# esteinig/sketchy

Measured on AMD Instinct MI355X. Metric: reads/sec streamed (s=10000,k=16,40k-genome ref), higher is better.
Workload: dtype u64

## Files before the change

include/sketchy_hip.h:

```cpp
#ifndef SKETCHY_HIP_H
#define SKETCHY_HIP_H

#include <stddef.h>
#include <stdint.h>

#ifdef __cplusplus
extern "C" {
#endif

#define SKX_OK 0
#define SKX_ERR_INVALID (-1)
#define SKX_ERR_NO_DEVICE (-2)
#define SKX_ERR_HIP (-3)
#define SKX_ERR_UNSORTED (-4)
#define SKX_ERR_CAPACITY (-5)
#define SKX_ERR_COMM (-6)
#define SKX_ERR_UNSUPPORTED (-7)

#define SKX_MAX_K 32u
#define SKX_MAX_TOP 64u
#define SKX_MAX_SPECIES 64u
#define SKX_MAX_FEATURES 64u
#define SKX_MAX_TABLE_SUM ((1ull << 54) - 1)

typedef struct skx_ref skx_ref;
typedef struct skx_stream skx_stream;
typedef struct skx_comm skx_comm;

const char *skx_last_error(void);
const char *skx_version(void);
int skx_device_count(void);
int skx_device_info(int device, char *name, size_t name_cap, int *compute_units, uint64_t *total_mem);
int skx_device_pci_bus_id(int device, char *bus_id, size_t cap);

#define SKX_COMM_TIMEOUT_EXIT 86
int skx_set_option(const char *name, uint64_t value);
int skx_get_option(const char *name, uint64_t *value);

int skx_ref_create(skx_ref **out, int device, uint32_t k, uint64_t seed, uint32_t s, uint32_t stride, uint32_t n_genomes,
                   const uint64_t *hashes, const uint32_t *col_len);
int skx_ref_create_multi(skx_ref **out, int device, uint32_t k, uint64_t seed, uint32_t s, uint32_t stride, uint32_t n_species,
                         const uint32_t *n_genomes, const uint64_t *const *hashes, const uint32_t *const *col_len);
int skx_ref_n_genomes(const skx_ref *ref, uint32_t *n_genomes);
int skx_ref_n_species(const skx_ref *ref, uint32_t *n_species);
int skx_ref_species_genomes(const skx_ref *ref, uint32_t species, uint32_t *n_genomes);
int skx_ref_sketch_size(const skx_ref *ref, uint32_t *s, uint32_t *stride);
int skx_ref_kmer_filter(const skx_ref *ref, uint64_t *n_keys, uint64_t *table_bytes);
int skx_ref_rare_index(const skx_ref *ref, uint64_t *n_keys, uint64_t *n_rare_keys, uint64_t *n_postings, uint64_t *bytes);
int skx_ref_patterns(const skx_ref *ref, uint64_t *n_long_lists, uint64_t *n_patterns, uint64_t *n_pattern_lists, uint64_t *bytes);
int skx_ref_static_dense(const skx_ref *ref, int *is_static, uint64_t *n_hashes);
int skx_ref_pass_bytes(const skx_ref *ref, uint64_t *bytes);
int skx_ref_set_genotypes(skx_ref *ref, uint32_t n_features, const uint32_t *codes);
int skx_ref_n_features(const skx_ref *ref, uint32_t *n_features);
void skx_ref_destroy(skx_ref *ref);

int skx_stream_create(skx_stream **out, const skx_ref *ref, uint32_t top_k, uint32_t max_batch_reads,
                      uint64_t max_batch_bases);
int skx_stream_push(skx_stream *st, const uint8_t *bases, const uint64_t *offsets, uint32_t n_reads,
                    uint32_t *topk_idx, uint64_t *topk_sum, uint32_t *per_read_shared, uint64_t *sketches,
                    uint32_t *sketch_len);
int skx_stream_push_device(skx_stream *st, const uint8_t *d_bases, const uint64_t *d_offsets, uint32_t n_reads,
                           uint64_t n_bases, uint32_t *d_topk_idx, uint64_t *d_topk_sum);
int skx_stream_enqueue_device(skx_stream *st, const uint8_t *d_bases, const uint64_t *d_offsets, uint32_t n_reads,
                              uint64_t n_bases, uint32_t *d_topk_idx, uint64_t *d_topk_sum);
int skx_stream_flush(skx_stream *st);
int skx_stream_set_packed_input(skx_stream *st, int on);
uint64_t skx_pack_bases(const uint8_t *ascii, uint64_t n, uint8_t *packed, uint64_t nibble_pos);
uint64_t skx_pack_line(const uint8_t *ascii, uint64_t n, uint8_t *packed, uint64_t nibble_pos, uint64_t *consumed);
int skx_stream_sync(skx_stream *st);
int skx_stream_submit(skx_stream *st, const uint8_t *bases, const uint64_t *offsets, uint32_t n_reads,
                      uint32_t *topk_idx, uint64_t *topk_sum, uint64_t *ticket);
int skx_stream_wait(skx_stream *st, uint64_t ticket);
int skx_stream_drain(skx_stream *st);
int skx_stream_bind_consensus(skx_stream *st, uint32_t *codes_out);
int skx_stream_bind_changes(skx_stream *st, uint32_t cap, uint32_t *n_events, uint32_t *ev_read, uint32_t *ev_idx, uint64_t *ev_sum,
                            uint32_t *ev_codes);
int skx_stream_table(skx_stream *st, uint64_t *cum);
int skx_stream_table_add(skx_stream *st, const uint64_t *add);
int skx_stream_reset(skx_stream *st);
int skx_stream_reads(const skx_stream *st, uint64_t *n_reads);
#define SKX_N_STATS 18
int skx_stream_stats(skx_stream *st, uint64_t *out, uint32_t n_out);
int skx_stream_rank(skx_stream *st, uint32_t top_k, uint32_t *idx, uint64_t *sum);
void skx_stream_destroy(skx_stream *st);

#define SKX_N_STAGES 5
int skx_stream_set_profiling(skx_stream *st, int enabled);
int skx_stream_profile(skx_stream *st, double *ms, uint64_t *launches);
int skx_stream_scan_alone(skx_stream *st, uint32_t reps, double *ms_avg);

int skx_sketch_reads(int device, uint32_t k, uint64_t seed, uint32_t s, const uint8_t *bases,
                     const uint64_t *offsets, uint32_t n_reads, uint64_t *sketches, uint32_t *sketch_len);
int skx_sketch_groups(int device, uint32_t k, uint64_t seed, uint32_t s, const uint8_t *bases, const uint64_t *offsets,
                      uint32_t n_records, const uint32_t *group_first, uint32_t n_groups,
                      uint64_t *sketches, uint32_t *sketch_len, uint64_t *valid_kmers);
int skx_sketch_groups_counts(int device, uint32_t k, uint64_t seed, uint32_t s, const uint8_t *bases, const uint64_t *offsets,
                             uint32_t n_records, const uint32_t *group_first, uint32_t n_groups, uint64_t *sketches,
                             uint32_t *sketch_len, uint64_t *valid_kmers, uint32_t *counts);
int skx_common_hashes(const skx_ref *ref, const uint64_t *query, const uint32_t *query_len, uint32_t n_query,
                      uint32_t q_stride, uint32_t *common);
int skx_rank_sketches(const skx_ref *ref, const uint64_t *query, const uint32_t *query_len, uint32_t n_query, uint32_t q_stride,
                      uint32_t top_k, uint32_t *top_idx, uint32_t *top_shared, uint32_t *common);
int skx_predict_groups(const skx_ref *ref, const uint8_t *bases, const uint64_t *offsets, uint32_t n_records,
                       const uint32_t *group_first, uint32_t n_groups, uint32_t top_k,
                       uint32_t *top_idx, uint32_t *top_shared, uint64_t *sketches, uint32_t *sketch_len, uint64_t *valid_kmers);
int skx_consensus_rows(const skx_ref *ref, const uint32_t *idx, uint64_t n_rows, uint32_t top_k, uint32_t *codes_out);

int skx_changes_rows(int device, const uint32_t *rows, uint64_t n_rows, uint32_t width, uint64_t cap, uint64_t *n_events,
                     uint64_t *ev_row);

#define SKX_COMM_ID_BYTES 128
int skx_comm_unique_id(uint8_t id[SKX_COMM_ID_BYTES]);
int skx_comm_create(skx_comm **out, int device, int rank, int n_ranks, const uint8_t id[SKX_COMM_ID_BYTES]);
int skx_comm_n_ranks(const skx_comm *comm, int *n_ranks);
int skx_stream_allreduce(skx_stream *st, skx_comm *comm);
void skx_comm_destroy(skx_comm *comm);

int skx_dev_malloc(int device, void **d_ptr, size_t bytes);
int skx_dev_free(int device, void *d_ptr);
int skx_dev_upload(int device, void *d_dst, const void *h_src, size_t bytes);
int skx_dev_download(int device, void *h_dst, const void *d_src, size_t bytes);
int skx_dev_synchronize(int device);
int skx_dev_mem_info(int device, uint64_t *free_bytes, uint64_t *total_bytes);
int skx_host_alloc(int device, void **h_ptr, size_t bytes);
int skx_host_free(int device, void *h_ptr);

#ifdef __cplusplus
}
#endif
#endif
```

sketchy_amd/_lib.py:

```python
import ctypes as C
import os

_HERE = os.path.dirname(os.path.abspath(__file__))
LIB_PATH = os.environ.get("SKX_LIB_PATH") or os.path.join(_HERE, "libsketchy_hip.so")

OK = 0
ERR_INVALID, ERR_NO_DEVICE, ERR_HIP, ERR_UNSORTED, ERR_CAPACITY, ERR_COMM, ERR_UNSUPPORTED = -1, -2, -3, -4, -5, -6, -7
N_STAGES = 5
STAGE_NAMES = ("sketch", "dictionary", "scan", "transpose", "rank")
COMM_ID_BYTES = 128
MAX_K = 32
MAX_TOP = 64
MAX_SPECIES = 64
MAX_FEATURES = 64
MAX_TABLE_SUM = (1 << 54) - 1

_vp, _u32, _u64, _i, _sz = C.c_void_p, C.c_uint32, C.c_uint64, C.c_int, C.c_size_t
_pp = C.POINTER(C.c_void_p)
SYMBOLS = [
    ("skx_last_error", C.c_char_p, []),
    ("skx_version", C.c_char_p, []),
    ("skx_device_count", _i, []),
    ("skx_device_info", _i, [_i, C.c_char_p, _sz, C.POINTER(_i), C.POINTER(_u64)]),
    ("skx_device_pci_bus_id", _i, [_i, C.c_char_p, _sz]),
    ("skx_set_option", _i, [C.c_char_p, _u64]),
    ("skx_get_option", _i, [C.c_char_p, C.POINTER(_u64)]),
    ("skx_ref_kmer_filter", _i, [_vp, C.POINTER(_u64), C.POINTER(_u64)]),
    ("skx_ref_rare_index", _i, [_vp, C.POINTER(_u64), C.POINTER(_u64), C.POINTER(_u64), C.POINTER(_u64)]),
    ("skx_ref_patterns", _i, [_vp, C.POINTER(_u64), C.POINTER(_u64), C.POINTER(_u64), C.POINTER(_u64)]),
    ("skx_ref_static_dense", _i, [_vp, C.POINTER(C.c_int), C.POINTER(_u64)]),
    ("skx_ref_create", _i, [_pp, _i, _u32, _u64, _u32, _u32, _u32, _vp, _vp]),
    ("skx_ref_create_multi", _i, [_pp, _i, _u32, _u64, _u32, _u32, _u32, _vp, _vp, _vp]),
    ("skx_ref_sketch_size", _i, [_vp, C.POINTER(_u32), C.POINTER(_u32)]),
    ("skx_ref_n_genomes", _i, [_vp, C.POINTER(_u32)]),
    ("skx_ref_n_species", _i, [_vp, C.POINTER(_u32)]),
    ("skx_ref_species_genomes", _i, [_vp, _u32, C.POINTER(_u32)]),
    ("skx_ref_pass_bytes", _i, [_vp, C.POINTER(_u64)]),
    ("skx_ref_set_genotypes", _i, [_vp, _u32, _vp]),
    ("skx_ref_n_features", _i, [_vp, C.POINTER(_u32)]),
    ("skx_ref_destroy", None, [_vp]),
    ("skx_stream_create", _i, [_pp, _vp, _u32, _u32, _u64]),
    ("skx_stream_push", _i, [_vp, _vp, _vp, _u32, _vp, _vp, _vp, _vp, _vp]),
    ("skx_stream_push_device", _i, [_vp, _vp, _vp, _u32, _u64, _vp, _vp]),
    ("skx_stream_enqueue_device", _i, [_vp, _vp, _vp, _u32, _u64, _vp, _vp]),
    ("skx_stream_flush", _i, [_vp]),
    ("skx_stream_set_packed_input", _i, [_vp, _i]),
    ("skx_pack_bases", _u64, [_vp, _u64, _vp, _u64]),
    ("skx_pack_line", _u64, [_vp, _u64, _vp, _u64, C.POINTER(_u64)]),
    ("skx_stream_sync", _i, [_vp]),
    ("skx_stream_submit", _i, [_vp, _vp, _vp, _u32, _vp, _vp, C.POINTER(_u64)]),
    ("skx_stream_wait", _i, [_vp, _u64]),
    ("skx_stream_drain", _i, [_vp]),
    ("skx_stream_bind_consensus", _i, [_vp, _vp]),
    ("skx_stream_bind_changes", _i, [_vp, _u32, _vp, _vp, _vp, _vp, _vp]),
    ("skx_stream_table", _i, [_vp, _vp]),
    ("skx_stream_table_add", _i, [_vp, _vp]),
    ("skx_stream_reset", _i, [_vp]),
    ("skx_stream_reads", _i, [_vp, C.POINTER(_u64)]),
    ("skx_stream_stats", _i, [_vp, C.POINTER(_u64), _u32]),
    ("skx_stream_rank", _i, [_vp, _u32, _vp, _vp]),
    ("skx_stream_destroy", None, [_vp]),
    ("skx_stream_set_profiling", _i, [_vp, _i]),
    ("skx_stream_profile", _i, [_vp, C.POINTER(C.c_double), C.POINTER(_u64)]),
    ("skx_stream_scan_alone", _i, [_vp, C.c_uint32, C.POINTER(C.c_double)]),
    ("skx_sketch_reads", _i, [_i, _u32, _u64, _u32, _vp, _vp, _u32, _vp, _vp]),
    ("skx_sketch_groups", _i, [_i, _u32, _u64, _u32, _vp, _vp, _u32, _vp, _u32, _vp, _vp, _vp]),
    ("skx_sketch_groups_counts", _i, [_i, _u32, _u64, _u32, _vp, _vp, _u32, _vp, _u32, _vp, _vp, _vp, _vp]),
    ("skx_common_hashes", _i, [_vp, _vp, _vp, _u32, _u32, _vp]),
    ("skx_rank_sketches", _i, [_vp, _vp, _vp, _u32, _u32, _u32, _vp, _vp, _vp]),
    ("skx_consensus_rows", _i, [_vp, _vp, _u64, _u32, _vp]),
    ("skx_changes_rows", _i, [_i, _vp, _u64, _u32, _u64, C.POINTER(_u64), _vp]),
    ("skx_predict_groups", _i, [_vp, _vp, _vp, _u32, _vp, _u32, _u32, _vp, _vp, _vp, _vp, _vp]),
    ("skx_comm_unique_id", _i, [_vp]),
    ("skx_comm_create", _i, [_pp, _i, _i, _i, _vp]),
    ("skx_comm_n_ranks", _i, [_vp, C.POINTER(_i)]),
    ("skx_stream_allreduce", _i, [_vp, _vp]),
    ("skx_comm_destroy", None, [_vp]),
    ("skx_dev_malloc", _i, [_i, _pp, _sz]),
    ("skx_dev_free", _i, [_i, _vp]),
    ("skx_dev_upload", _i, [_i, _vp, _vp, _sz]),
    ("skx_dev_download", _i, [_i, _vp, _vp, _sz]),
    ("skx_dev_synchronize", _i, [_i]),
# ... 34 lines not shown
```

sketchy_amd/api.py:

```python
import ctypes as C

import numpy as np

from . import _lib


def _p(a):
    return None if a is None else a.ctypes.data_as(C.c_void_p)


def pack_reads(bases, offsets, first_nibble=0):
    L = _lib.load()
    bases = np.ascontiguousarray(bases, np.uint8)
    offsets = np.ascontiguousarray(offsets, np.uint64)
    n = len(offsets) - 1
    packed = np.zeros((first_nibble + len(bases) + 1) // 2 + 1, np.uint8)
    out = np.zeros(n + 1, np.uint64)
    pos = int(first_nibble)
    out[0] = pos
    for r in range(n):
        a, b = int(offsets[r]), int(offsets[r + 1])
        if b > a:
            pos = int(L.skx_pack_bases(bases[a:b].ctypes.data_as(C.c_void_p), b - a, _p(packed), pos))
        out[r + 1] = pos
# ... 39 lines not shown
    for f in range(n_feat):
        col = [r[f] for r in rows]
        distinct = sorted(set(col), key=key)
        rank = {v: i for i, v in enumerate(distinct)}
        codes[:, f] = [rank[v] for v in col]
        values.append(distinct)
    return codes, values


class ReferenceSketch:

    def __init__(self, hashes, col_len=None, k=16, seed=0, device=0, s=None):
        L = _lib.load()
        many = isinstance(hashes, (list, tuple))
        mats = [np.ascontiguousarray(h, np.uint64) for h in (hashes if many else [hashes])]
        if any(m.ndim != 2 for m in mats) or len({m.shape[1] for m in mats}) != 1:
            raise ValueError("hashes must be [n_genomes, s] (one matrix per species, all with the same s)")
        lens = col_len if many else [col_len]
        lens = [None] * len(mats) if lens is None else list(lens)
        lens = [np.full(m.shape[0], m.shape[1], np.uint32) if c is None else np.ascontiguousarray(c, np.uint32)
                for m, c in zip(mats, lens)]
        self.species = [int(m.shape[0]) for m in mats]
        self.n_species = len(mats)
        self.n_genomes, self.stride = sum(self.species), int(mats[0].shape[1])
        self.s = self.stride if s is None else int(s)
        self.k, self.seed, self.device = int(k), int(seed), int(device)
        h = C.c_void_p()
        if self.n_species == 1:
            _lib.check(L.skx_ref_create(C.byref(h), device, self.k, self.seed, self.s, self.stride, self.n_genomes, _p(mats[0]), _p(lens[0])))
        else:
            ng = (C.c_uint32 * self.n_species)(*self.species)
            hp = (C.c_void_p * self.n_species)(*[m.ctypes.data for m in mats])
            cp = (C.c_void_p * self.n_species)(*[c.ctypes.data for c in lens])
            _lib.check(L.skx_ref_create_multi(C.byref(h), device, self.k, self.seed, self.s, self.stride, self.n_species, ng, hp, cp))
        self._h = h

    @property
    def kmer_filter(self):
        n, b = C.c_uint64(0), C.c_uint64(0)
        _lib.check(_lib.load().skx_ref_kmer_filter(self._h, C.byref(n), C.byref(b)))
        return n.value, b.value

    @property
    def rare_index(self):
        v = [C.c_uint64(0) for _ in range(4)]
        _lib.check(_lib.load().skx_ref_rare_index(self._h, *[C.byref(x) for x in v]))
        return dict(zip(("keys", "rare_keys", "postings", "bytes"), [x.value for x in v]))

    @property
    def patterns(self):
        v = [C.c_uint64(0) for _ in range(4)]
        _lib.check(_lib.load().skx_ref_patterns(self._h, *[C.byref(x) for x in v]))
        return dict(zip(("long_lists", "patterns", "pattern_lists", "bytes"), [x.value for x in v]))

    @property
    def static_dense(self):
        f, n = C.c_int(0), C.c_uint64(0)
        _lib.check(_lib.load().skx_ref_static_dense(self._h, C.byref(f), C.byref(n)))
        return bool(f.value), n.value

    @property
    def pass_bytes(self) -> int:
        b = C.c_uint64(0)
        _lib.check(_lib.load().skx_ref_pass_bytes(self._h, C.byref(b)))
        return b.value

    def common_hashes(self, query, query_len=None) -> np.ndarray:
        query = np.ascontiguousarray(query, np.uint64)
        nq, stride = query.shape
        query_len = np.full(nq, stride, np.uint32) if query_len is None else np.ascontiguousarray(query_len, np.uint32)
        out = np.zeros((nq, self.n_genomes), np.uint32)
        _lib.check(_lib.load().skx_common_hashes(self._h, _p(query), _p(query_len), nq, stride, _p(out)))
        return out

    def rank_sketches(self, query, query_len=None, top=1, want_common=False):
        query = np.ascontiguousarray(query, np.uint64)
        if query.ndim != 2:
            raise ValueError("query must be [n_query, stride]")
        nq, stride = query.shape
        query_len = np.full(nq, stride, np.uint32) if query_len is None else np.ascontiguousarray(query_len, np.uint32)
        if query_len.shape != (nq,):
            raise ValueError("query_len must hold one length per query row")
        top = int(top)
        idx = np.zeros((nq, self.n_species, max(top, 0)), np.uint32)
        shared = np.zeros_like(idx)
        common = np.zeros((nq, self.n_genomes), np.uint32) if want_common else None
        if stride == 0:
            if query_len.any():
                raise ValueError("query_len exceeds the stride of the query rows")
            query, stride = np.zeros((max(nq, 1), 1), np.uint64), 1
        _lib.check(_lib.load().skx_rank_sketches(self._h, _p(query), _p(query_len), nq, stride, top, _p(idx), _p(shared),
                                                 _p(common) if want_common else None))
        return (idx, shared, common) if want_common else (idx, shared)

    def predict_groups(self, bases, offsets, group_first, top=1, want_sketches=False, want_valid_kmers=False):
        bases = np.ascontiguousarray(bases, np.uint8)
        offsets = np.ascontiguousarray(offsets, np.uint64)
        group_first = np.ascontiguousarray(group_first, np.uint32)
        if offsets.ndim != 1 or len(offsets) < 1 or group_first.ndim != 1 or len(group_first) < 1:
            raise ValueError("offsets and group_first are 1-D with at least one entry")
        n, ng = len(offsets) - 1, len(group_first) - 1
        top = int(top)
        idx = np.zeros((ng, self.n_species, max(top, 0)), np.uint32)
        shared = np.zeros_like(idx)
        sk = np.zeros((ng, self.s), np.uint64) if want_sketches else None
        sl = np.zeros(ng, np.uint32) if want_sketches else None
# ... 112 lines not shown

    def flush(self):
        _lib.check(_lib.load().skx_stream_flush(self._h))

    def set_packed_input(self, on=True):
        _lib.check(_lib.load().skx_stream_set_packed_input(self._h, int(bool(on))))

    def sync(self):
        _lib.check(_lib.load().skx_stream_sync(self._h))

    def submit(self, h_bases, h_offsets, n_reads, h_topk_idx=None, h_topk_sum=None, consensus=None, changes=None) -> int:
        self._bind(consensus, changes)
        t = C.c_uint64(0)
        _lib.check(_lib.load().skx_stream_submit(self._h, h_bases, h_offsets, n_reads, h_topk_idx, h_topk_sum, C.byref(t)))
        return t.value

    def wait(self, ticket):
        _lib.check(_lib.load().skx_stream_wait(self._h, ticket))

    def drain(self):
        _lib.check(_lib.load().skx_stream_drain(self._h))

    def table(self) -> np.ndarray:
        cum = np.zeros(self.ref.n_genomes, np.uint64)
        _lib.check(_lib.load().skx_stream_table(self._h, _p(cum)))
        return cum

    def table_add(self, add):
        add = np.ascontiguousarray(add, np.uint64)
        assert len(add) == self.ref.n_genomes
        _lib.check(_lib.load().skx_stream_table_add(self._h, _p(add)))

    def reset(self):
        _lib.check(_lib.load().skx_stream_reset(self._h))

    @property
    def reads(self) -> int:
        n = C.c_uint64(0)
        _lib.check(_lib.load().skx_stream_reads(self._h, C.byref(n)))
        return n.value

    def rank(self, top=None):
        top = self.top if top is None else int(top)
        shape = (top,) if self.ref.n_species == 1 else (self.ref.n_species, top)
        idx, sm = np.zeros(shape, np.uint32), np.zeros(shape, np.uint64)
        _lib.check(_lib.load().skx_stream_rank(self._h, top, _p(idx), _p(sm)))
        return idx, sm

    def consensus(self, top=None) -> np.ndarray:
        idx, _ = self.rank(top)
        return self.ref.consensus_rows(idx)

    def stats(self):
        v = (C.c_uint64 * 18)()
        _lib.check(_lib.load().skx_stream_stats(self._h, v, 18))
        names = ("last_pairs", "last_passes", "dictionary_size", "reads_block_sketcher", "passes", "passes_lean_scan",
                 "pair_capacity", "live_rank_groups", "reads_split_over_waves", "read_segments", "row_pool_grown",
                 "passes_shared", "groups_unshared", "query_rows", "query_rows_grown", "dictionary_dense", "batches_compact", "batches_full")
        return dict(zip(names, [int(x) for x in v]))

    def set_profiling(self, on=True):
        _lib.check(_lib.load().skx_stream_set_profiling(self._h, int(on)))

    def profile(self):
        ms = (C.c_double * _lib.N_STAGES)()
        n = (C.c_uint64 * _lib.N_STAGES)()
        _lib.check(_lib.load().skx_stream_profile(self._h, ms, n))
        return {name: dict(ms=ms[i], launches=int(n[i])) for i, name in enumerate(_lib.STAGE_NAMES)}

    def scan_alone(self, reps=3) -> float:
        ms = C.c_double(0)
        _lib.check(_lib.load().skx_stream_scan_alone(self._h, int(reps), C.byref(ms)))
        return ms.value

    def allreduce(self, comm):
        _lib.check(_lib.load().skx_stream_allreduce(self._h, comm._h))

    def close(self):
        if getattr(self, "_h", None):
            _lib.load().skx_stream_destroy(self._h)
            self._h = None

    def __del__(self):
        try:
            self.close()
        except Exception:
            pass


class Comm:

    @staticmethod
    def unique_id() -> bytes:
        buf = (C.c_uint8 * _lib.COMM_ID_BYTES)()
        _lib.check(_lib.load().skx_comm_unique_id(buf))
        return bytes(buf)

    def __init__(self, device, rank, n_ranks, uid: bytes):
        buf = (C.c_uint8 * _lib.COMM_ID_BYTES).from_buffer_copy(uid)
        h = C.c_void_p()
        _lib.check(_lib.load().skx_comm_create(C.byref(h), device, rank, n_ranks, buf))
        self._h = h

    @property
    def n_ranks(self) -> int:
        n = C.c_int(0)
        _lib.check(_lib.load().skx_comm_n_ranks(self._h, C.byref(n)))
        return n.value

    def close(self):
        if getattr(self, "_h", None):
# ... 92 lines not shown
```

sketchy_amd/csrc/skx_capi.hip:

```cpp
#include <dlfcn.h>
#include <hip/hip_runtime.h>
#include <rccl/rccl.h>

#include <unistd.h>

#include <algorithm>
#include <atomic>
#include <chrono>
#include <cmath>
#include <condition_variable>
#include <cstdarg>
#include <cstdio>
#include <cstdlib>
#include <cstring>
#include <mutex>
#include <string>
#include <thread>
#include <unordered_map>
#include <vector>

#include "sketchy_hip.h"
#include "skx_common.hpp"
#include "skx_kernels.hpp"

// ... 184 lines not shown
        return SKX_OK;
    }
    return fail(SKX_ERR_INVALID, "unknown option '%s'", name);
}
SKX_API int skx_get_option(const char* name, uint64_t* value) {
    if (!name || !value) return fail(SKX_ERR_INVALID, "NULL argument");
    if (!strcmp(name, "kmer_prefilter")) { *value = g_kmer_prefilter; return SKX_OK; }
    if (!strcmp(name, "filter_bits_per_hash")) { *value = g_filter_bits_per_hash; return SKX_OK; }
    if (!strcmp(name, "stream_query_rows")) { *value = g_stream_query_rows; return SKX_OK; }
    if (!strcmp(name, "stream_coalesce")) { *value = g_stream_coalesce; return SKX_OK; }
    if (!strcmp(name, "comm_timeout_ms")) { *value = g_comm_timeout_ms; return SKX_OK; }
    if (!strcmp(name, "rank_lanes")) { *value = g_rank_lanes; return SKX_OK; }
    if (!strcmp(name, "rare_hash_genomes")) { *value = g_rare_hash_genomes; return SKX_OK; }
    if (!strcmp(name, "reuse_membership")) { *value = g_reuse_membership; return SKX_OK; }
    return fail(SKX_ERR_INVALID, "unknown option '%s'", name);
}

struct skx_ref {
    int device = 0;
    u32 k = 0, s = 0 , s_read = 0 ;
    u32 n_genomes = 0 , n_tiles = 0, n_pad = 0, rb = 0, n_bands = 0;
    u64 seed = 0;
    u32 n_species = 0;
    std::vector<u32> sp_n, sp_g0, sp_real0;
    u32 min_species = 0;
    u32 max_species = 0;
    u32 *d_sp_g0 = nullptr, *d_sp_n = nullptr, *d_grp_sp = nullptr;
    u32* d_real2pad = nullptr;
    u64* d_mat = nullptr;
    u64 *d_lo = nullptr, *d_hi = nullptr;
    u64 max_ref = 0;
    bool any = false;
    u32 n_exc = 0;
    u32* d_exc_g = nullptr;
    u64* d_exc_h = nullptr;
    u64* d_filt = nullptr;
    u32 filt_shift = 0;
    u64 filt_bits = 0, n_distinct = 0;
    u32* d_kf = nullptr;
    u32 kf_shift = 0, kf_keys = 0;
    u64* d_kt_key = nullptr;
    u32 *d_kt_cnt = nullptr, *d_kt_off = nullptr, *d_post = nullptr;
    u32 kt_mask = 0, rare_max = 0;
    u64 n_keys = 0, n_rare_keys = 0, n_postings = 0;
    u64* d_mlong = nullptr;
    u64* d_mlongT = nullptr;
    u32 *d_lid = nullptr, *d_lslot = nullptr;
    u64 n_long = 0;
    u32 n_lw = 0;
    u32 *d_prec = nullptr, *d_pat_rep = nullptr, *d_npat = nullptr;
    u64* d_pm = nullptr;
    u32 n_pat = 0;
    u64 n_pat_lists = 0;
    bool rare_direct = false;
    u64* d_qs = nullptr;
    u32* d_nsd = nullptr;
    u32* d_win_s = nullptr;
    u32 n_sd = 0;
    bool static_dense = false;
    u32* d_srow = nullptr;
    u32* d_seg = nullptr;
    u32* d_segw = nullptr;
    u32 sd_tail0 = 0;
    u64 n_forced_rare = 0;
    u32* d_codes = nullptr;
    u32 n_features = 0;
    skx::RareIndex rare_index() const {
        skx::RareIndex ri{d_kt_key, d_kt_off, d_kt_cnt, d_post, kt_mask, d_mlong, d_lid, d_lslot, n_pad / 64, d_mlongT, n_lw};
        ri.prec = d_prec; ri.pat_rep = d_pat_rep; ri.pm = d_pm; ri.d_npat = d_npat; ri.n_pat = n_pat;
        if (static_dense) { ri.qs = d_qs; ri.n_sd = n_sd; ri.srow = d_srow; ri.tail0 = sd_tail0; }
        return ri;
    }
    skx::KmerFilter kmer_filter() const { return skx::KmerFilter{d_kf, kf_shift}; }
    skx::Species species() const { return skx::Species{d_sp_g0, d_sp_n, d_grp_sp, n_species}; }
};

static void ref_free(skx_ref* r) {
    if (!r) return;
    (void)hipSetDevice(r->device);
    (void)hipFree(r->d_mat); (void)hipFree(r->d_lo); (void)hipFree(r->d_hi);
    (void)hipFree(r->d_exc_g); (void)hipFree(r->d_exc_h); (void)hipFree(r->d_filt); (void)hipFree(r->d_kf);
    (void)hipFree(r->d_sp_g0); (void)hipFree(r->d_sp_n); (void)hipFree(r->d_grp_sp); (void)hipFree(r->d_real2pad);
    (void)hipFree(r->d_kt_key); (void)hipFree(r->d_kt_cnt); (void)hipFree(r->d_kt_off); (void)hipFree(r->d_post);
    (void)hipFree(r->d_mlong); (void)hipFree(r->d_mlongT); (void)hipFree(r->d_lid); (void)hipFree(r->d_lslot);
    (void)hipFree(r->d_prec); (void)hipFree(r->d_pat_rep); (void)hipFree(r->d_npat); (void)hipFree(r->d_pm);
    (void)hipFree(r->d_qs); (void)hipFree(r->d_nsd); (void)hipFree(r->d_win_s);
    (void)hipFree(r->d_srow); (void)hipFree(r->d_seg); (void)hipFree(r->d_segw); (void)hipFree(r->d_codes);
    delete r;
}

static const u32 kGroupGenomes = skx::kRankWords * 64u;

static const u32 kPatMax = 16384;
static const u32 kPatGroupMin = 4;
static void build_patterns(skx_ref* r) {
    static const int pat_env = skx::knob("SKX_PATTERNS") ? atoi(skx::knob("SKX_PATTERNS")) : 1;
    if (!pat_env || !r->d_mlong || r->n_long < 64 || r->n_long >= 0x7FFFFFFFull) return;
    const u32 n_long = (u32)r->n_long, n_gw = r->n_pad / 64;
    u32 *d_sig = nullptr, *d_pat_of = nullptr, *d_done = nullptr;
    u64* d_content = nullptr;
    auto drop = [&]() {
        (void)hipFree(r->d_prec); (void)hipFree(r->d_pat_rep); (void)hipFree(r->d_npat); (void)hipFree(r->d_pm);
        r->d_prec = r->d_pat_rep = r->d_npat = nullptr; r->d_pm = nullptr; r->n_pat = 0; r->n_pat_lists = 0;
        (void)hipGetLastError();
    };
    bool ok = hipMalloc(&d_sig, (size_t)n_long * 4) == hipSuccess && hipMalloc(&d_content, (size_t)n_long * 8) == hipSuccess;
    try {
        std::vector<u32> sig(n_long), pat_of(n_long, 0xFFFFFFFFu), rep;
        std::vector<u64> content(n_long);
        if (ok) {
            skx::launch_list_sig(nullptr, r->d_lslot, n_long, r->d_kt_off, r->d_kt_cnt, r->d_post, d_sig, d_content);
            ok = hipGetLastError() == hipSuccess && hipMemcpy(sig.data(), d_sig, (size_t)n_long * 4, hipMemcpyDeviceToHost) == hipSuccess &&
                 hipMemcpy(content.data(), d_content, (size_t)n_long * 8, hipMemcpyDeviceToHost) == hipSuccess;
        }
        if (ok) {
            struct Exact { u32 count = 0, first = 0, sig = 0; };
            struct Group { u32 size = 0, best_count = 0, best_first = 0; };
            std::unordered_map<u64, Exact> exact;
            std::unordered_map<u32, Group> groups;
            exact.reserve(n_long);
            for (u32 i = 0; i < n_long; ++i) {
                Exact& e = exact[content[i] ^ ((u64)sig[i] * 0xD6E8FEB86659FD93ull)];
                if (!e.count) { e.first = i; e.sig = sig[i]; }
                e.count += 1;
                groups[sig[i]].size += 1;
            }
            for (const auto& kv : exact) {
                const Exact& e = kv.second;
                Group& g = groups[e.sig];
                if (e.count > g.best_count || (e.count == g.best_count && e.first < g.best_first)) { g.best_count = e.count; g.best_first = e.first; }
            }
            std::vector<std::pair<u32, u32>> order;
            for (const auto& kv : groups) if (kv.second.size >= kPatGroupMin) order.push_back({kv.second.size, kv.first});
            std::sort(order.begin(), order.end(), [](const std::pair<u32, u32>& a, const std::pair<u32, u32>& b) { return a.first != b.first ? a.first > b.first : a.second < b.second; });
            if (order.size() > kPatMax) order.resize(kPatMax);
            std::unordered_map<u32, u32> pat_of_sig;
            for (const auto& o : order) { pat_of_sig[o.second] = (u32)rep.size(); rep.push_back(groups[o.second].best_first); }
            for (u32 i = 0; i < n_long; ++i) { const auto it = pat_of_sig.find(sig[i]); if (it != pat_of_sig.end()) pat_of[i] = it->second; }
            ok = !rep.empty();
        }
        const u32 n_pat = (u32)rep.size(), n_pw = (n_pat + 63) / 64;
        size_t mem_free = 0, mem_total = 0;
        (void)hipMemGetInfo(&mem_free, &mem_total);
        ok = ok && ((size_t)n_long * skx::pat_record_words() * 4 + (size_t)n_pw * r->n_pad * 8) <= mem_free / 8;
        ok = ok && hipMalloc(&d_pat_of, (size_t)n_long * 4) == hipSuccess && hipMalloc(&d_done, 4) == hipSuccess &&
             hipMalloc(&r->d_pat_rep, (size_t)n_pat * 4) == hipSuccess && hipMalloc(&r->d_npat, 16) == hipSuccess &&
             hipMalloc(&r->d_prec, (size_t)n_long * skx::pat_record_words() * 4) == hipSuccess &&
             hipMalloc(&r->d_pm, (size_t)n_pw * r->n_pad * 8) == hipSuccess &&
             hipMemcpy(d_pat_of, pat_of.data(), (size_t)n_long * 4, hipMemcpyHostToDevice) == hipSuccess &&
             hipMemcpy(r->d_pat_rep, rep.data(), (size_t)n_pat * 4, hipMemcpyHostToDevice) == hipSuccess &&
             hipMemset(d_done, 0, 4) == hipSuccess;
        if (ok) {
            const u32 words[4] = {n_pat, 0u, (n_pat + 63u) & ~63u, n_pat};
            ok = hipMemcpy(r->d_npat, words, 16, hipMemcpyHostToDevice) == hipSuccess;
        }
        if (ok) {
            skx::launch_pat_exceptions(nullptr, r->d_mlong, n_gw, n_long, d_pat_of, r->d_pat_rep, r->d_prec, d_done);
            skx::launch_pat_matrix(nullptr, r->d_mlong, r->d_pat_rep, n_pat, n_gw, r->d_pm, r->n_pad);
            u32 done = 0;
            ok = hipGetLastError() == hipSuccess && hipDeviceSynchronize() == hipSuccess && hipMemcpy(&done, d_done, 4, hipMemcpyDeviceToHost) == hipSuccess;
            ok = ok && (u64)done * 8 >= n_long;
            if (ok) { r->n_pat = n_pat; r->n_pat_lists = done; }
        }
    } catch (const std::bad_alloc&) { ok = false; }
    (void)hipFree(d_sig); (void)hipFree(d_content); (void)hipFree(d_pat_of); (void)hipFree(d_done);
    if (!ok) drop();
}

static void build_static_dense(skx_ref* r, const std::vector<u64>& exc_h, const std::vector<u64>* spmask) {
    static const int sd_env = skx::knob("SKX_STATIC_DENSE") ? atoi(skx::knob("SKX_STATIC_DENSE")) : 1;
    if (!sd_env || !r->d_kt_key || !r->rare_direct) return;
    const u64 slots = (u64)r->kt_mask + 1;
    const u32 n_sp = r->n_species;
    const u64 cap_sp = (u64)191 * r->s / std::max<u32>(r->rb, 1u), cap = std::min<u64>(131072, cap_sp * n_sp);
    u64* d_keys = nullptr;
    u32 *d_slots = nullptr, *d_n = nullptr;
    bool ok = cap >= 1 && hipMalloc(&d_keys, (cap + 1) * 8) == hipSuccess && hipMalloc(&d_slots, (cap + 1) * 4) == hipSuccess &&
              hipMalloc(&d_n, 4) == hipSuccess && hipMemset(d_n, 0, 4) == hipSuccess;
    u32 n = 0;
    if (ok) {
        skx::launch_collect_dense(nullptr, r->d_kt_key, r->d_kt_off, slots, d_keys, d_slots, d_n, (u32)cap);
        ok = hipGetLastError() == hipSuccess && hipMemcpy(&n, d_n, 4, hipMemcpyDeviceToHost) == hipSuccess && n <= cap;
    }
    std::vector<u64> keys(n);
    std::vector<u32> kslot(n);
    ok = ok && (n == 0 || (hipMemcpy(keys.data(), d_keys, (size_t)n * 8, hipMemcpyDeviceToHost) == hipSuccess &&
                           hipMemcpy(kslot.data(), d_slots, (size_t)n * 4, hipMemcpyDeviceToHost) == hipSuccess));
    (void)hipFree(d_keys); (void)hipFree(d_slots); (void)hipFree(d_n);
    if (!ok) { (void)hipGetLastError(); return; }
    try {
        std::vector<std::vector<std::pair<u64, u32>>> per(n_sp);
        for (u32 i = 0; i < n; ++i) {
            u32 sp = 0;
            if (n_sp > 1) {
                const u64 m = spmask ? (*spmask)[kslot[i]] : 0;
                if (m == 0 || (m & (m - 1)) != 0) return;
                sp = (u32)__builtin_ctzll(m);
            }
            per[sp].push_back({keys[i], kslot[i]});
        }
        std::vector<u64> ex(exc_h);
        std::sort(ex.begin(), ex.end());
        ex.erase(std::unique(ex.begin(), ex.end()), ex.end());
        std::vector<u32> seg(2 * n_sp), segw(2 * n_sp);
        u32 row = 0;
        for (u32 sp = 0; sp < n_sp; ++sp) {
            if (per[sp].size() > cap_sp) return;
            std::sort(per[sp].begin(), per[sp].end());
            seg[2 * sp] = row; seg[2 * sp + 1] = (u32)per[sp].size();
            segw[2 * sp] = row / 64; segw[2 * sp + 1] = (row + (u32)per[sp].size() + 63) / 64;
            row = (row + (u32)per[sp].size() + 63u) & ~63u;
        }
        const u32 t0 = row, n_sd = ex.empty() ? (n_sp ? seg[2 * (n_sp - 1)] + seg[2 * (n_sp - 1) + 1] : 0u) : t0 + (u32)ex.size();
        std::vector<u64> qs(std::max<u32>(n_sd, 1u), 0xFFFFFFFFFFFFFFFFull);
        std::vector<u32> srow(slots, 0xFFFFFFFFu);
        for (u32 sp = 0; sp < n_sp; ++sp)
            for (u32 i = 0; i < per[sp].size(); ++i) { qs[seg[2 * sp] + i] = per[sp][i].first; srow[per[sp][i].second] = seg[2 * sp] + i; }
        for (u32 i = 0; i < ex.size(); ++i) qs[t0 + i] = ex[i];
        const u32 n_bt = r->n_bands * r->n_tiles;
// ... 200 lines not shown
                     hipMemset(d_over, 0, 4) == hipSuccess;
                if (ok && n_species > 1) ok = hipMalloc(&d_spm, slots * 8) == hipSuccess && hipMemset(d_spm, 0, slots * 8) == hipSuccess;
                if (!ok) break;
                skx::launch_rare_count(nullptr, r->d_mat, mat_elems, r->d_kt_key, r->d_kt_cnt, (u32)(slots - 1), d_over, d_spm, r->d_grp_sp, s);
                u32 over = 0;
                ok = hipGetLastError() == hipSuccess && hipMemcpy(&over, d_over, 4, hipMemcpyDeviceToHost) == hipSuccess;
                if (ok && !over) break;
                drop();
                (void)hipFree(d_spm); d_spm = nullptr;
                if (attempt == 3) ok = false;
            }
            std::vector<u64> spm;
            if (ok && r->d_kt_key) try {
                std::vector<u32> cnt(slots), off(slots);
                ok = hipMemcpy(cnt.data(), r->d_kt_cnt, slots * 4, hipMemcpyDeviceToHost) == hipSuccess;
                if (ok && d_spm) { spm.resize(slots); ok = hipMemcpy(spm.data(), d_spm, slots * 8, hipMemcpyDeviceToHost) == hipSuccess; }
                (void)hipFree(d_spm); d_spm = nullptr;
                u64 total = 0, keys = 0, rare = 0, long_keys = 0, forced = 0;
                for (u64 i = 0; ok && i < slots; ++i) {
                    const bool multi = !spm.empty() && (spm[i] & (spm[i] - 1)) != 0 && cnt[i] > rare_max && cnt[i] <= (1u << 18);
                    if (cnt[i] && (cnt[i] <= rare_max || multi)) { off[i] = (u32)total; total += cnt[i]; ++rare; long_keys += cnt[i] > 8u ? 1 : 0; forced += multi ? 1 : 0; }
                    else off[i] = 0xFFFFFFFFu;
                    keys += cnt[i] ? 1 : 0;
                }
                r->n_forced_rare = forced;
                ok = ok && total < 0xFFFFFFF0ull;
                ok = ok && hipMalloc(&r->d_kt_off, slots * 4) == hipSuccess && hipMalloc(&r->d_post, std::max<u64>(total, 1) * 4) == hipSuccess &&
                     hipMalloc(&d_cursor, slots * 4) == hipSuccess && hipMemset(d_cursor, 0, slots * 4) == hipSuccess &&
                     hipMemcpy(r->d_kt_off, off.data(), slots * 4, hipMemcpyHostToDevice) == hipSuccess;
                if (ok) {
                    skx::launch_rare_fill(nullptr, r->d_mat, mat_elems, s, r->d_kt_key, r->d_kt_off, d_cursor, r->d_post, (u32)(slots - 1));
                    ok = hipGetLastError() == hipSuccess && hipDeviceSynchronize() == hipSuccess;
                }
                if (ok) { r->kt_mask = (u32)(slots - 1); r->rare_max = rare_max; r->n_keys = keys; r->n_rare_keys = rare; r->n_postings = total; }
                static const int mlong_env = skx::knob("SKX_LONG_ROWS") ? atoi(skx::knob("SKX_LONG_ROWS")) : 1;
                if (ok && mlong_env) {
                    std::vector<u32> lid(slots, 0xFFFFFFFFu), lslot;
                    for (u64 i = 0; i < slots; ++i)
                        if (off[i] != 0xFFFFFFFFu && cnt[i] > 8u) { lid[i] = (u32)lslot.size(); lslot.push_back((u32)i); }
                    const u64 n_long = lslot.size(), row_bytes = (u64)r->n_pad / 8;
                    size_t mem_free = 0, mem_total = 0;
                    (void)hipMemGetInfo(&mem_free, &mem_total);
                    bool lok = n_long > 0 && n_long * row_bytes <= mem_free / 8 &&
                               hipMalloc(&r->d_mlong, n_long * row_bytes) == hipSuccess && hipMemset(r->d_mlong, 0, n_long * row_bytes) == hipSuccess &&
                               hipMalloc(&r->d_lid, slots * 4) == hipSuccess && hipMalloc(&r->d_lslot, n_long * 4) == hipSuccess &&
                               hipMemcpy(r->d_lid, lid.data(), slots * 4, hipMemcpyHostToDevice) == hipSuccess &&
                               hipMemcpy(r->d_lslot, lslot.data(), n_long * 4, hipMemcpyHostToDevice) == hipSuccess;
                    if (lok) {
                        skx::launch_mlong_build(nullptr, r->d_lslot, (u32)n_long, r->d_kt_off, r->d_kt_cnt, r->d_post, r->d_mlong, r->n_pad / 64);
                        lok = hipGetLastError() == hipSuccess && hipDeviceSynchronize() == hipSuccess;
                    }
                    if (lok) r->n_long = n_long;
                    if (lok) build_patterns(r);
                    const bool mostly_patterns = lok && r->d_prec && r->n_pat_lists * 10 >= n_long * 9;
                    static const int mlongt_env = skx::knob("SKX_LONG_ROWS_T") ? atoi(skx::knob("SKX_LONG_ROWS_T")) : 1;
                    if (lok && mlongt_env && (!mostly_patterns || mlongt_env == 2)) {
                        const u32 n_lw = (u32)((n_long + 63) / 64);
                        const u64 t_bytes = (u64)r->n_pad * n_lw * 8;
                        (void)hipMemGetInfo(&mem_free, &mem_total);
                        if (t_bytes <= mem_free / 8 && hipMalloc(&r->d_mlongT, t_bytes) == hipSuccess) {
                            skx::launch_mlong_transpose(nullptr, r->d_mlong, (u32)n_long, r->n_pad / 64, r->d_mlongT, n_lw);
                            if (hipGetLastError() == hipSuccess && hipDeviceSynchronize() == hipSuccess) r->n_lw = n_lw;
                            else { (void)hipFree(r->d_mlongT); r->d_mlongT = nullptr; }
                        } else r->d_mlongT = nullptr;
                        (void)hipGetLastError();
                    }
                    else if (!lok) { (void)hipFree(r->d_mlong); (void)hipFree(r->d_lid); (void)hipFree(r->d_lslot); r->d_mlong = nullptr; r->d_lid = r->d_lslot = nullptr; r->n_long = 0; (void)hipGetLastError(); }
                }
                r->rare_direct = ok && (r->d_mlong != nullptr || long_keys == 0);
            } catch (const std::bad_alloc&) {
                (void)hipFree(r->d_mlong); (void)hipFree(r->d_mlongT); (void)hipFree(r->d_lid); (void)hipFree(r->d_lslot);
                r->d_mlong = r->d_mlongT = nullptr; r->d_lid = r->d_lslot = nullptr; r->n_long = 0; r->n_lw = 0;
                (void)hipFree(r->d_prec); (void)hipFree(r->d_pat_rep); (void)hipFree(r->d_npat); (void)hipFree(r->d_pm);
                r->d_prec = r->d_pat_rep = r->d_npat = nullptr; r->d_pm = nullptr; r->n_pat = 0; r->n_pat_lists = 0;
                r->rare_direct = false;
                ok = false;
            }
            (void)hipFree(d_over); (void)hipFree(d_cursor);
            (void)hipFree(d_spm);
            if (!ok) { drop(); r->rare_direct = false; }
            else build_static_dense(r, exc_h, spm.empty() ? nullptr : &spm);
        }
    }
    const u32 pf_mode = skx::knob("SKX_KMER_PREFILTER") ? (u32)atoi(skx::knob("SKX_KMER_PREFILTER")) : g_kmer_prefilter.load();
    static const u32 kf_bits = skx::knob("SKX_KF_BITS") ? (u32)std::max(1, atoi(skx::knob("SKX_KF_BITS"))) : 8u;
    const u64 kf_auto_bits = 8ull << 15;
    if (k == 16 && any && pf_mode) {
        u32* d_n = nullptr;
        RCHK(hipMalloc(&d_n, 4));
        RCHK(hipMemset(d_n, 0, 4));
        skx::launch_kmer_filter_build(nullptr, seed, max_ref, r->d_filt, r->filt_shift, d_n, nullptr, 0);
        RCHK(hipGetLastError());
        RCHK(hipMemcpy(&r->kf_keys, d_n, 4, hipMemcpyDeviceToHost));
        (void)hipFree(d_n);
        auto table_lg_words = [&](u32 bits) {
            u32 lg = 10;
            while (lg < 27 && (32ull << lg) < (u64)bits * r->kf_keys) ++lg;
            return lg;
        };
        u32 lg_words = table_lg_words(kf_bits);
        if (pf_mode >= 2 && (32ull << lg_words) > kf_auto_bits) {
            lg_words = table_lg_words(std::max(1u, kf_bits / 2));
            if ((32ull << lg_words) > kf_auto_bits) { lg_words = 0; r->kf_keys = 0; }
        }
        if (lg_words) {
            r->kf_shift = 32u - lg_words;
            RCHK(hipMalloc(&r->d_kf, (size_t)4 << lg_words));
            RCHK(hipMemset(r->d_kf, 0, (size_t)4 << lg_words));
            skx::launch_kmer_filter_build(nullptr, seed, max_ref, r->d_filt, r->filt_shift, nullptr, r->d_kf, r->kf_shift);
            RCHK(hipGetLastError());
            RCHK(hipDeviceSynchronize());
        }
    }
#undef RCHK
    *out = r;
    return SKX_OK;
}
SKX_API int skx_ref_create(skx_ref** out, int device, uint32_t k, uint64_t seed, uint32_t s, uint32_t stride, uint32_t n_genomes,
                           const uint64_t* hashes, const uint32_t* col_len) {
    if (!out || !hashes || !col_len) return fail(SKX_ERR_INVALID, "NULL argument");
    *out = nullptr;
    if (s < 1 || stride < 1 || n_genomes < 1)
        return fail(SKX_ERR_INVALID, "empty reference (s=%u, stride=%u, n_genomes=%u)", s, stride, n_genomes);
    return skx_ref_create_multi(out, device, k, seed, s, stride, 1, &n_genomes, &hashes, &col_len);
}
SKX_API int skx_ref_sketch_size(const skx_ref* ref, uint32_t* s, uint32_t* stride) {
    if (!ref) return fail(SKX_ERR_INVALID, "NULL argument");
    if (s) *s = ref->s_read;
    if (stride) *stride = ref->s;
    return SKX_OK;
}
SKX_API int skx_ref_n_genomes(const skx_ref* ref, uint32_t* n_genomes) {
    if (!ref || !n_genomes) return fail(SKX_ERR_INVALID, "NULL argument");
    *n_genomes = ref->n_genomes;
    return SKX_OK;
}
SKX_API int skx_ref_n_species(const skx_ref* ref, uint32_t* n_species) {
    if (!ref || !n_species) return fail(SKX_ERR_INVALID, "NULL argument");
    *n_species = ref->n_species;
    return SKX_OK;
}
SKX_API int skx_ref_species_genomes(const skx_ref* ref, uint32_t species, uint32_t* n_genomes) {
    if (!ref || !n_genomes) return fail(SKX_ERR_INVALID, "NULL argument");
    if (species >= ref->n_species) return fail(SKX_ERR_INVALID, "species %u outside 0..%u", species, ref->n_species - 1);
    *n_genomes = ref->sp_n[species];
    return SKX_OK;
}
SKX_API int skx_ref_kmer_filter(const skx_ref* ref, uint64_t* n_keys, uint64_t* table_bytes) {
    if (!ref) return fail(SKX_ERR_INVALID, "NULL argument");
    if (n_keys) *n_keys = ref->d_kf ? ref->kf_keys : 0;
    if (table_bytes) *table_bytes = ref->d_kf ? (4ull << (32u - ref->kf_shift)) : 0;
    return SKX_OK;
}
SKX_API int skx_ref_rare_index(const skx_ref* ref, uint64_t* n_keys, uint64_t* n_rare_keys, uint64_t* n_postings, uint64_t* bytes) {
    if (!ref) return fail(SKX_ERR_INVALID, "NULL argument");
    const bool on = ref->d_kt_key != nullptr;
    if (n_keys) *n_keys = on ? ref->n_keys : 0;
    if (n_rare_keys) *n_rare_keys = on ? ref->n_rare_keys : 0;
    if (n_postings) *n_postings = on ? ref->n_postings : 0;
    if (bytes) *bytes = on ? ((u64)ref->kt_mask + 1) * 16 + std::max<u64>(ref->n_postings, 1) * 4 + (ref->d_mlong ? ref->n_long * (ref->n_pad / 8 + 4) + ((u64)ref->kt_mask + 1) * 4 : 0) + (ref->d_mlongT ? (u64)ref->n_pad * ref->n_lw * 8 : 0) : 0;
    return SKX_OK;
}
SKX_API int skx_ref_patterns(const skx_ref* ref, uint64_t* n_long_lists, uint64_t* n_patterns, uint64_t* n_pattern_lists, uint64_t* bytes) {
    if (!ref) return fail(SKX_ERR_INVALID, "NULL argument");
    if (n_long_lists) *n_long_lists = ref->d_mlong ? ref->n_long : 0;
    if (n_patterns) *n_patterns = ref->d_prec ? ref->n_pat : 0;
    if (n_pattern_lists) *n_pattern_lists = ref->d_prec ? ref->n_pat_lists : 0;
    if (bytes) *bytes = ref->d_prec ? ref->n_long * skx::pat_record_words() * 4 + (u64)((ref->n_pat + 63) / 64) * ref->n_pad * 8 + (u64)ref->n_pat * 4 : 0;
    return SKX_OK;
}
SKX_API int skx_ref_static_dense(const skx_ref* ref, int* is_static, uint64_t* n_hashes) {
    if (!ref) return fail(SKX_ERR_INVALID, "NULL argument");
    if (is_static) *is_static = ref->static_dense ? 1 : 0;
    if (n_hashes) *n_hashes = ref->static_dense ? ref->n_sd : 0;
    return SKX_OK;
}
SKX_API int skx_ref_pass_bytes(const skx_ref* ref, uint64_t* bytes) {
    if (!ref || !bytes) return fail(SKX_ERR_INVALID, "NULL argument");
    *bytes = 8ull * ref->s * ref->n_genomes;
    return SKX_OK;
}

SKX_API int skx_ref_set_genotypes(skx_ref* ref, uint32_t n_features, const uint32_t* codes) {
    if (!ref || !codes) return fail(SKX_ERR_INVALID, "skx_ref_set_genotypes: NULL argument");
    if (n_features < 1 || n_features > SKX_MAX_FEATURES)
        return fail(SKX_ERR_INVALID, "skx_ref_set_genotypes: n_features=%u outside 1..%u", n_features, SKX_MAX_FEATURES);
    if (ref->d_codes) return fail(SKX_ERR_INVALID, "skx_ref_set_genotypes: the reference already has a genotype table");
    SKXCHK(use_device(ref->device));
    std::vector<u32> padded((size_t)ref->n_pad * n_features, 0u);
    for (u32 sp = 0; sp < ref->n_species; ++sp)
        memcpy(padded.data() + (size_t)ref->sp_g0[sp] * n_features, codes + (size_t)ref->sp_real0[sp] * n_features,
               (size_t)ref->sp_n[sp] * n_features * 4);
    u32* d = nullptr;
    HIPCHK(hipMalloc(&d, padded.size() * 4));
    const hipError_t e = hipMemcpy(d, padded.data(), padded.size() * 4, hipMemcpyHostToDevice);
    if (e != hipSuccess) { (void)hipFree(d); return fail(SKX_ERR_HIP, "skx_ref_set_genotypes: %s", hipGetErrorString(e)); }
    ref->d_codes = d;
    ref->n_features = n_features;
    return SKX_OK;
}
SKX_API int skx_ref_n_features(const skx_ref* ref, uint32_t* n_features) {
    if (!ref || !n_features) return fail(SKX_ERR_INVALID, "NULL argument");
    *n_features = ref->n_features;
    return SKX_OK;
}
SKX_API void skx_ref_destroy(skx_ref* ref) { ref_free(ref); }

struct TimedSpan { int stage; hipEvent_t a, b; };

static const int kGroupMax = skx::kPairBaseMax + 1;
struct ChangeOut {
    u32 cap = 0;
    u32 n_batch = 0;
    u32 *n_events = nullptr, *ev_read = nullptr, *ev_idx = nullptr;
    u64* ev_sum = nullptr;
    u32* ev_codes = nullptr;
    bool codes = false;
};
struct PendingBatch {
    bool valid = false;
    int side = 0;
// ... 53 lines not shown
struct skx_stream {
    const skx_ref* ref = nullptr;
    int device = 0;
    hipStream_t hs0 = nullptr, hs = nullptr, hs2 = nullptr;
    hipStream_t hs1 = nullptr;
    bool tail_pass = false;
    hipEvent_t ev_main[kSides] = {};
    int depth = 2;
    bool shared_queues = false;
    int buf = 0;
    hipEvent_t ev_dict[2] = {nullptr, nullptr}, ev_front[2] = {nullptr, nullptr}, ev_back[2] = {nullptr, nullptr};
    hipEvent_t ev_sketch[kSides] = {};
    hipEvent_t ev_skread[kSides] = {};
    bool sk_reader_pending[kSides] = {};
    int side = 0;
    PendingBatch pend[kGroupMax];
    int n_pend = 0;
    u32 group_cap = 1;
    u32 clean_groups = 0;
    double ppr_est = 0.0, qpr_est = 0.0;
    int side_next = 0;
    bool front_pending[2] = {false, false};
    bool back_pending[2] = {false, false};
    hipEvent_t ev_pslot[3] = {nullptr, nullptr, nullptr};
    bool pslot_pending[3] = {false, false, false};
    int pslot = 0;
    hipEvent_t ev_pairq[2] = {nullptr, nullptr};
    bool pairq_pending[2] = {false, false};
    bool packed = false;
    u32 top_k = 0, max_reads = 0, sk_stride = 0;
    u64 max_bases = 0;
    u32 pcap = 0;
    u32 qcap = 0;
    u64* d_qd = nullptr;
    u32 *d_qrow = nullptr, *d_sslot = nullptr, *d_qinfo = nullptr, *d_qloc = nullptr, *d_cls_bsum = nullptr;
    u32* d_nd_hs = nullptr;
    u32* h_lcount = nullptr;
    u32 lcount_seq = 0, lcount_seen = 0, lcount_floor = 0;
    u32* h_nq_sink = nullptr;
    u32* h_nd = nullptr;
    u32 *d_rowcnt = nullptr;
    u32 *d_gain = nullptr;
    u32 *d_gain_s = nullptr;
    u32 *d_candslot = nullptr;
    u32 *d_candmask = nullptr;
    uint2 *d_lrow = nullptr;
    u32 *d_nlrow = nullptr, *d_gain_l = nullptr, *d_cbase = nullptr, *d_cwl = nullptr, *d_ncwl = nullptr;
    u64 *d_cw = nullptr;
    u64 *d_inb = nullptr, *d_hit = nullptr;
    skx::LongRows long_rows() const { return skx::LongRows{d_lrow, d_nlrow, qcap + 128, d_inb, ref->n_lw}; }
    bool use_pat = false;
    u32 *d_hist = nullptr, *d_nprow = nullptr;
    u64* d_pcw = nullptr;
    u32 npat_pad = 0;
    skx::PatRows pat_rows() const { return skx::PatRows{d_hist, npat_pad, d_gain_l, d_nprow}; }
    skx::RareIndex rare_index() const {
        skx::RareIndex ri = ref->rare_index();
        if (!use_pat) { ri.prec = nullptr; ri.n_pat = 0; }
        if (!static_dense) { ri.qs = nullptr; ri.n_sd = 0; }
        return ri;
    }
    u32 *d_cbad = nullptr, *d_nqc = nullptr;
    u32 *d_spc_g0 = nullptr, *d_spc_grp = nullptr;
    u32 n_pad_c = 0, n_grp_c = 0, cand_seq = 0;
    struct PassSet {
        u64 *tab = nullptr;
        u32 *cand = nullptr;
        u64 *tabc = nullptr;
        u32 *ncand = nullptr;
        u32 *mode = nullptr, *any_full = nullptr, *nqc_total = nullptr;
        u64 *mc = nullptr;
        u64 *mqc = nullptr;
        u64 *rowany_c = nullptr;
        u32 *grp_any_c = nullptr;
        u32 *smap = nullptr;
        u32 *pair_qc = nullptr;
        u32 *nd = nullptr;
        u32 *h_pub = nullptr;
    } ps[2];
    struct PassChains {
        bool pending = false, ranked = false, has_cand = false, update_table = false, forced_full = false, legacy = false;
        SubPass subs[kGroupMax];
        int n_sub = 0, b = 0, slot = 0;
        u32 P = 0, nq_rows = 0, seq = 0;
        u64 nq_est = 0;
    } pcq[2];
    int pc_head = 0, pc_n = 0;
    bool hint_all_overflow = false;
    u32 hint_seq = 0;
    u32 passes_since_fresh = 0;
    bool fresh_table = true;
    u32 legacy_run = 0;
    u64 batches_compact = 0, batches_full = 0;
    bool have_split_hint = false;
    double nd_frac = 1.0;
    u32 qcap_max = 0;
    bool qcap_auto = false;
    u64 qrows_grown = 0;
    u32 coalesce = 1;
    u32 rpass = 0;
    u64 reads_total = 0;
    uint8_t* d_bases = nullptr;
    u64* d_offsets = nullptr;
    u64* d_sk = nullptr;
    u32 *d_len = nullptr, *d_cnt = nullptr, *d_poff = nullptr;
    bool side_ready[kSides] = {};
    u64* sd_sk[kSides] = {};
    u64 pool_cap[kSides] = {};
// ... 86 lines not shown
    u64 groups_unshared = 0;
    u64 last_pairs = 0, last_passes = 0, total_passes = 0, lean_passes = 0;
    struct Staged {
        bool pending = false;
        bool in_flight = false;
        bool dropped = false;
        u32 n_reads = 0;
        u64 n_bases = 0, ticket = 0;
        u32* out_idx = nullptr;
        u64* out_sum = nullptr;
        u32* out_cons = nullptr;
        u32* d_cons = nullptr;
        ChangeOut out_chg;
        ChangeOut d_ev;
        u32* h_ev_n = nullptr;
        u32* d_rows_idx = nullptr;
        u64* d_rows_sum = nullptr;
        uint8_t* d_bases = nullptr;
        u64 *d_offsets = nullptr, *h_offsets = nullptr;
        hipEvent_t ev_copy = nullptr, ev_done = nullptr;
    } slot[kSlotsMax];
    u32 n_slots = 3;
    hipStream_t hs_copy = nullptr;
    u64 next_ticket = 0;
    u32* h_nq = nullptr;
    u32 hint_pairs[2] = {0, 0};
    double nq_per_pair = 1.0;
    bool have_hint = false;
    int profiling = 0;
    std::vector<TimedSpan> spans;
    std::vector<hipEvent_t> ev_pool;
    double ms[SKX_N_STAGES] = {0, 0, 0, 0, 0};
    u64 launches[SKX_N_STAGES] = {0, 0, 0, 0, 0};
};

static void free_side(skx_stream* st, int i);
static void free_lane(skx_stream* st, int i);
static void stream_free(skx_stream* st) {
    if (!st) return;
    (void)hipSetDevice(st->device);
    if (st->hs0) (void)hipStreamSynchronize(st->hs0);
    if (st->hs1) (void)hipStreamSynchronize(st->hs1);
    if (st->hs) (void)hipStreamSynchronize(st->hs);
    if (st->hs2) (void)hipStreamSynchronize(st->hs2);
    for (int i = 1; i < skx_stream::kRankLanes; ++i)
        if (st->lane[i].s) (void)hipStreamSynchronize(st->lane[i].s);
    for (int i = 0; i < kSides; ++i) (void)hipFree(st->sd_rows[i]);
    void* ptrs[] = {st->d_bases, st->d_offsets, st->d_pair_h[0], st->d_pair_h[1],
                    st->d_q[0], st->d_q[1], st->d_pair_r[0], st->d_pair_r[1], st->d_pair_q[0], st->d_pair_q[1],
                    st->d_poff_pass[0], st->d_poff_pass[1], st->d_poff_pass[2], st->d_pair_r[2], st->d_nq[0], st->d_nq[1], st->d_win[0], st->d_win[1], st->d_m, st->d_mint, st->d_mq[0], st->d_mq[1],
                    st->d_topk_idx, st->d_topk_sum, st->d_cons, st->d_ev.n_events, st->d_ev.ev_read, st->d_ev.ev_idx, st->d_ev.ev_sum, st->d_ev.ev_codes, st->d_tab_tmp, st->d_rank_idx, st->d_rank_sum, st->d_bsum, st->d_grp_any[0],
                    st->d_grp_any[1], st->d_hbuf, st->d_wb[0], st->d_wb[1], st->d_rowany[0], st->d_rowany[1], st->d_mqext,
                    st->d_qd, st->d_qrow, st->d_sslot, st->d_qinfo, st->d_qloc, st->d_cls_bsum, st->d_nd_hs,
                    st->d_rowcnt, st->d_gain, st->d_gain_s, st->d_candslot, st->d_candmask, st->d_lrow, st->d_nlrow, st->d_gain_l, st->d_cbase, st->d_cwl, st->d_ncwl, st->d_cw, st->d_cbad, st->d_nqc, st->d_spc_g0, st->d_spc_grp, st->d_inb, st->d_hit, st->d_hist, st->d_nprow, st->d_pcw, st->d_ms[0], st->d_ms[1], st->d_mdirty_s};
    for (auto& q : st->ps) {
        for (void* x : {(void*)q.tab, (void*)q.cand, (void*)q.tabc, (void*)q.ncand, (void*)q.mode, (void*)q.any_full, (void*)q.nqc_total, (void*)q.mc, (void*)q.mqc,
                        (void*)q.rowany_c, (void*)q.grp_any_c, (void*)q.smap, (void*)q.pair_qc, (void*)q.nd}) (void)hipFree(x);
        if (q.h_pub) (void)hipHostFree(q.h_pub);
    }
    for (auto& t : st->d_tab) (void)hipFree(t);
    for (int i = 0; i < skx_stream::kRankLanes; ++i) free_lane(st, i);
    for (int i = 1; i < skx_stream::kRankLanes; ++i)
        if (st->own_lane_stream && st->lane[i].s) (void)hipStreamDestroy(st->lane[i].s);
    for (void* p : ptrs) (void)hipFree(p);
    if (st->h_poff) (void)hipHostFree(st->h_poff);
    if (st->h_offsets) (void)hipHostFree(st->h_offsets);
    if (st->h_nq) (void)hipHostFree(st->h_nq);
    if (st->h_nd) (void)hipHostFree(st->h_nd);
    if (st->h_nq_sink) (void)hipHostFree(st->h_nq_sink);
    if (st->h_lcount) (void)hipHostFree(st->h_lcount);
    if (st->h_chk_base) (void)hipHostFree(st->h_chk_base);
    for (int i = 0; i < kSides; ++i) {
        free_side(st, i);
        if (st->ev_main[i]) (void)hipEventDestroy(st->ev_main[i]);
    }
    if (!st->shared_queues && st->hs1 && st->hs1 != st->hs0) (void)hipStreamDestroy(st->hs1);
    (void)hipFree(st->d_ht[0]); (void)hipFree(st->d_ht[1]); (void)hipFree(st->d_dict_ctr[0]); (void)hipFree(st->d_dict_ctr[1]);
    (void)hipFree(st->d_slot_off); (void)hipFree(st->d_bcount); (void)hipFree(st->d_bbase);
    (void)hipFree(st->d_btot);
    for (auto& sl : st->slot) {
        (void)hipFree(sl.d_bases); (void)hipFree(sl.d_offsets); (void)hipFree(sl.d_rows_idx); (void)hipFree(sl.d_rows_sum); (void)hipFree(sl.d_cons);
        (void)hipFree(sl.d_ev.n_events); (void)hipFree(sl.d_ev.ev_read); (void)hipFree(sl.d_ev.ev_idx); (void)hipFree(sl.d_ev.ev_sum); (void)hipFree(sl.d_ev.ev_codes);
        if (sl.h_ev_n) (void)hipHostFree(sl.h_ev_n);
        if (sl.h_offsets) (void)hipHostFree(sl.h_offsets);
        if (sl.ev_copy) (void)hipEventDestroy(sl.ev_copy);
        if (sl.ev_done) (void)hipEventDestroy(sl.ev_done);
    }
    if (st->hs_copy) (void)hipStreamDestroy(st->hs_copy);
    for (auto& sp : st->spans) { (void)hipEventDestroy(sp.a); (void)hipEventDestroy(sp.b); }
    for (auto ev : st->ev_pool) (void)hipEventDestroy(ev);
    for (int i = 0; i < 2; ++i) {
        if (st->ev_dict[i]) (void)hipEventDestroy(st->ev_dict[i]);
        if (st->ev_pairq[i]) (void)hipEventDestroy(st->ev_pairq[i]);
        if (st->ev_front[i]) (void)hipEventDestroy(st->ev_front[i]);
        if (st->ev_back[i]) (void)hipEventDestroy(st->ev_back[i]);
    }
    for (int i = 0; i < kSides; ++i) {
        if (st->ev_sketch[i]) (void)hipEventDestroy(st->ev_sketch[i]);
        if (st->ev_skread[i]) (void)hipEventDestroy(st->ev_skread[i]);
    }
    for (auto ev : st->ev_pslot)
        if (ev) (void)hipEventDestroy(ev);
    if (st->shared_queues) {
        release_queues(st->device);
    } else {
        if (st->hs2 && st->hs2 != st->hs && st->hs2 != st->hs0) (void)hipStreamDestroy(st->hs2);
        if (st->hs0 && st->hs0 != st->hs) (void)hipStreamDestroy(st->hs0);
// ... 350 lines not shown
    SCHK(hipMalloc(&st->d_slot_off, (size_t)st->ht_slots * 4));
    SCHK(hipMalloc(&st->d_btot, 256 * 4));
    SCHK(hipMalloc(&st->d_bcount, (size_t)skx::dict_buckets() * 4));
    SCHK(hipMemset(st->d_bcount, 0, (size_t)skx::dict_buckets() * 4));
    SCHK(hipMalloc(&st->d_bbase, (size_t)skx::dict_buckets() * 4));
    SCHK(hipHostMalloc((void**)&st->h_chk_base, kSides * 16 * 4, hipHostMallocCoherent));
    memset(st->h_chk_base, 0, kSides * 16 * 4);
    SCHK(use_side(st, 0));
    SCHK(hipHostMalloc((void**)&st->h_nq, 4 * 4, hipHostMallocCoherent));
    st->h_nq[0] = st->h_nq[1] = 0;
    st->h_nq[2] = 1; st->h_nq[3] = 1;
    SCHK(hipHostMalloc((void**)&st->h_nd, 4 * 4, hipHostMallocCoherent));
    memset(st->h_nd, 0, 4 * 4);
    SCHK(hipHostMalloc((void**)&st->h_nq_sink, 4 * 4, hipHostMallocCoherent));
    SCHK(hipHostMalloc((void**)&st->h_lcount, 4 * 4, hipHostMallocCoherent));
    memset(st->h_lcount, 0, 4 * 4);
    SCHK(hipMalloc(&st->d_nd_hs, 64));
    SCHK(hipMemset(st->d_nd_hs, 0, 64));
    if (ref->d_kt_key) {
        SCHK(hipMalloc(&st->d_qd, (size_t)st->pcap * 8));
        SCHK(hipMalloc(&st->d_qrow, (size_t)st->pcap * 4));
        SCHK(hipMalloc(&st->d_sslot, (size_t)st->pcap * 8));
        SCHK(hipMalloc(&st->d_qinfo, (size_t)st->pcap * 4));
        SCHK(hipMalloc(&st->d_qloc, (size_t)st->pcap * 4));
        SCHK(hipMalloc(&st->d_cls_bsum, ((size_t)st->pcap / 1024 + 2) * 4));
    }
    {
        const u32 nb = skx::kPassBatchesMax, cap = skx::kCandCap, rows_c = skx::kCandRows;
        st->n_pad_c = n_sp * cap;
        st->n_grp_c = st->n_pad_c / (skx::kRankWords * 64);
        SCHK(hipMalloc(&st->d_rowcnt, (size_t)nb * ((size_t)st->qcap + 128) * 4));
        SCHK(hipMalloc(&st->d_gain, (size_t)nb * n_pad * 4));
        if (ref->d_kt_key) SCHK(hipMalloc(&st->d_gain_s, (size_t)nb * n_pad * 4 * skx::gain_sparse_stride()));
        SCHK(hipMalloc(&st->d_candslot, (size_t)nb * n_pad * 4));
        SCHK(hipMalloc(&st->d_candmask, (size_t)n_pad * 4));
        if (ref->d_mlong) {
            SCHK(hipMalloc(&st->d_lrow, (size_t)nb * ((size_t)st->qcap + 128) * 8));
            SCHK(hipMalloc(&st->d_nlrow, skx::pass_counter_bytes()));
            SCHK(hipMalloc(&st->d_gain_l, (size_t)nb * n_pad * 4));
            SCHK(hipMalloc(&st->d_cw, (size_t)nb * (n_pad / 64) * 8));
            SCHK(hipMalloc(&st->d_cbase, (size_t)nb * (n_pad / 64) * 4));
            SCHK(hipMalloc(&st->d_cwl, (size_t)nb * st->n_pad_c * 4));
            SCHK(hipMalloc(&st->d_ncwl, 64));
            if (ref->d_mlongT) {
                SCHK(hipMalloc(&st->d_inb, (size_t)nb * ref->n_lw * 8));
                SCHK(hipMalloc(&st->d_hit, (size_t)nb * ref->n_lw * 8));
            }
            if (ref->d_prec && ref->n_pat && st->n_grp_c * skx::kRankWords <= skx::pat_words_max()) {
                st->use_pat = true;
                st->npat_pad = (ref->n_pat + 63u) & ~63u;
                SCHK(hipMalloc(&st->d_hist, (size_t)nb * st->npat_pad * 4));
                SCHK(hipMalloc(&st->d_nprow, skx::pass_counter_bytes()));
                SCHK(hipMalloc(&st->d_pcw, (size_t)nb * ref->n_pat * st->n_grp_c * skx::kRankWords * 8));
            }
        }
        SCHK(hipMalloc(&st->d_cbad, 64));
        SCHK(hipMalloc(&st->d_nqc, skx::pass_counter_bytes()));
        std::vector<u32> g0c(n_sp), grpc(st->n_grp_c);
        for (u32 i = 0; i < n_sp; ++i) g0c[i] = i * cap;
        for (u32 i = 0; i < st->n_grp_c; ++i) grpc[i] = i / (cap / (skx::kRankWords * 64));
        SCHK(hipMalloc(&st->d_spc_g0, (size_t)n_sp * 4));
        SCHK(hipMalloc(&st->d_spc_grp, (size_t)st->n_grp_c * 4));
        SCHK(hipMemcpy(st->d_spc_g0, g0c.data(), (size_t)n_sp * 4, hipMemcpyHostToDevice));
        SCHK(hipMemcpy(st->d_spc_grp, grpc.data(), (size_t)st->n_grp_c * 4, hipMemcpyHostToDevice));
        for (auto& q : st->ps) {
            SCHK(hipMalloc(&q.tab, (size_t)(nb + 1) * n_pad * 8));
            SCHK(hipMalloc(&q.cand, (size_t)nb * st->n_pad_c * 4));
            SCHK(hipMalloc(&q.tabc, (size_t)nb * st->n_pad_c * 8));
            SCHK(hipMalloc(&q.ncand, (size_t)nb * n_sp * 4));
            SCHK(hipMalloc(&q.mode, 64)); SCHK(hipMalloc(&q.any_full, 64)); SCHK(hipMalloc(&q.nqc_total, 64));
            SCHK(hipMemset(q.any_full, 0, 64));
            SCHK(hipMalloc(&q.mc, (size_t)nb * (rows_c / 64) * st->n_pad_c * 8));
            SCHK(hipMalloc(&q.mqc, (size_t)nb * st->n_grp_c * rows_c * skx::kRankWords * 8));
            SCHK(hipMalloc(&q.rowany_c, (size_t)nb * st->n_grp_c * (rows_c / 64) * 8));
            SCHK(hipMalloc(&q.grp_any_c, (size_t)nb * st->n_grp_c * 4 + 64));
            SCHK(hipMalloc(&q.smap, (size_t)nb * ((size_t)st->qcap + 128) * 4));
            SCHK(hipMalloc(&q.pair_qc, (size_t)st->pcap * 4));
            SCHK(hipMalloc(&q.nd, 64));
            SCHK(hipMemset(q.nd, 0, 64));
            SCHK(hipHostMalloc((void**)&q.h_pub, 32 * 4, hipHostMallocCoherent));
            memset(q.h_pub, 0, 32 * 4);
        }
    }
    SCHK(hipDeviceSynchronize());
#undef SCHK
    *out = st;
    return SKX_OK;
}

SKX_API int skx_stream_create(skx_stream** out, const skx_ref* ref, uint32_t top_k, uint32_t max_batch_reads,
                              uint64_t max_batch_bases) {
    if (!out || !ref) return fail(SKX_ERR_INVALID, "NULL argument");
    *out = nullptr;
    if (top_k > ref->min_species) return fail(SKX_ERR_INVALID, "top_k=%u exceeds n_genomes=%u", top_k, ref->min_species);
    if (top_k > SKX_MAX_TOP) return fail(SKX_ERR_INVALID, "top_k=%u exceeds SKX_MAX_TOP=%u", top_k, SKX_MAX_TOP);
    if (max_batch_reads < 1) return fail(SKX_ERR_INVALID, "max_batch_reads must be >= 1");
    const u64 longest = std::max<u64>(max_batch_bases, (u64)skx::kSketchCap);
    const u32 sk_stride = (u32)std::min<u64>(ref->s_read, longest);
    if (max_batch_bases >= (1ull << 32)) return fail(SKX_ERR_CAPACITY, "max_batch_bases must be below 2^32");
    return stream_create_internal(out, ref, top_k, max_batch_reads, max_batch_bases, sk_stride, 64, false, true);
}
SKX_API void skx_stream_destroy(skx_stream* st) { stream_free(st); }

static int flush_pending(skx_stream* st);
SKX_API int skx_stream_sync(skx_stream* st);
static hipEvent_t get_event(skx_stream* st) {
// ... 355 lines not shown
        st->cum_writer = nullptr;
    }
    if (update_table && !legacy) {
        Span sp(st, 4, hs);
        const u32 n_sp = ref->n_species, cap = skx::kCandCap, rows_c = skx::kCandRows;
        const u64* m_int = split ? st->d_mint : nullptr;
        HIPCHK(hipMemsetAsync(st->d_gain, 0, (size_t)n_sub * n_pad * 4, hs));
        if (P > 0) {
            SKXCHK(row_counts());
            skx::launch_gain_dense(hs, d_m, m_int, n_pad, d_nd, sdm ? ref->n_sd : q_bound, st->d_rowcnt, qstride, (u32)n_sub, st->d_gain,
                                   (sdm && ref->n_species > 1) ? ref->d_segw : nullptr, ref->d_grp_sp);
            if (split_dict) SKXCHK(rare_gains(hs));
        }
        skx::launch_pass_tables(hs, st->d_cum, st->d_gain, (split_dict && P > 0) ? st->d_gain_s : nullptr,
                                (long_rows && P > 0) ? st->d_gain_l : nullptr, (u32)n_sub, n_pad, ps.tab);
        st->d_cum = ps.tab + (size_t)n_sub * n_pad;
        static const int cand_env = skx::knob("SKX_CAND") ? atoi(skx::knob("SKX_CAND")) : 1;
        static const int hint_env = skx::knob("SKX_CAND_HINT") ? atoi(skx::knob("SKX_CAND_HINT")) : 1;
        (void)hint_env;
        all_forced = !cand_env;
        u32 force_full = all_forced ? 0xFFu : 0u;
        for (int i = 0; i < n_sub; ++i) if (subs[i].d_shared || subs[i].d_counts) force_full |= 1u << i;
        HIPCHK(hipMemsetAsync(st->d_cbad, 0, 64, hs));
        HIPCHK(hipMemsetAsync(st->d_nqc, 0, skx::pass_counter_bytes(), hs));
        const bool pat_rows = st->use_pat && long_rows && ranked && P > 0 && !all_forced;
        if (pat_rows) skx::launch_pat_nqc_init(hs, st->d_nqc, st->npat_pad);
        if (ranked) {
            HIPCHK(hipMemsetAsync(st->d_candmask, 0, (size_t)n_pad * 4, hs));
            skx::launch_cand_select(hs, ps.tab, n_pad, spc, (u32)n_sub, st->top_k, cap, ps.cand, st->d_candslot, ps.tabc, ps.ncand, st->d_cbad,
                                    st->d_candmask);
            HIPCHK(hipMemsetAsync(ps.grp_any_c, 0, (size_t)n_sub * st->n_grp_c * 4, hs));
            if (split_dict && P > 0 && !all_forced) {
                HIPCHK(hipMemsetAsync(ps.mqc, 0, (size_t)n_sub * st->n_grp_c * rows_c * skx::kRankWords * 8, hs));
                HIPCHK(hipMemsetAsync(ps.rowany_c, 0, (size_t)n_sub * st->n_grp_c * (rows_c / 64) * 8, hs));
                HIPCHK(hipMemset2DAsync(ps.smap, (size_t)qstride * 4, 0, (size_t)nq_rows * 4, (size_t)n_sub, hs));
                skx::launch_cand_sparse(hs, st->d_sslot, d_nd, q_bound, st->rare_index(), st->d_candmask, st->d_candslot, n_pad, st->d_cbad, (u32)n_sub, st->d_nqc,
                                        ps.smap, qstride, ps.mqc, (size_t)st->n_grp_c * rows_c * skx::kRankWords, rows_c, ps.rowany_c,
                                        st->n_grp_c * (rows_c / 64), ps.grp_any_c, st->n_grp_c, walk_scale);
                if (long_rows) {
                    const u32 n_gw = n_pad / 64;
                    HIPCHK(hipMemsetAsync(st->d_cw, 0, (size_t)n_sub * n_gw * 8, hs));
                    HIPCHK(hipMemsetAsync(st->d_cbase, 0xFF, (size_t)n_sub * n_gw * 4, hs));
                    HIPCHK(hipMemsetAsync(st->d_ncwl, 0, 64, hs));
                    skx::launch_cand_words(hs, ps.cand, st->n_pad_c, (u32)n_sub, n_gw, st->d_cw, st->d_cbase, st->d_cwl, st->d_ncwl);
                    if (st->d_hit) skx::launch_cand_hit(hs, ps.cand, st->n_pad_c, (u32)n_sub, st->d_cbad, st->rare_index(), st->d_inb, st->d_hit);
                    skx::launch_cand_long(hs, st->long_rows(), st->rare_index(), d_nd, st->d_cw, st->d_cbase, st->d_cwl, st->d_ncwl, st->n_pad_c,
                                          st->d_cbad, (u32)n_sub, st->d_nqc, ps.smap, qstride, ps.mqc, (size_t)st->n_grp_c * rows_c * skx::kRankWords,
                                          rows_c, ps.rowany_c, st->n_grp_c * (rows_c / 64), ps.grp_any_c, st->n_grp_c, walk_scale, st->d_hit);
                }
                if (pat_rows) {
                    const skx::RareIndex ri = st->rare_index();
                    skx::launch_cand_pat_rows(hs, ri, d_nd, st->d_candmask, st->d_candslot, n_pad, st->d_cbad, (u32)n_sub, st->d_pcw, ps.mqc,
                                              (size_t)st->n_grp_c * rows_c * skx::kRankWords, rows_c, ps.rowany_c, st->n_grp_c * (rows_c / 64), ps.grp_any_c,
                                              st->n_grp_c);
                    skx::launch_cand_pat_map(hs, st->long_rows(), st->pat_rows(), ri, d_nd, st->d_candmask, st->d_candslot, n_pad, st->d_cbad, (u32)n_sub,
                                             st->d_nqc, ps.smap, qstride, st->d_pcw, ps.mqc, (size_t)st->n_grp_c * rows_c * skx::kRankWords, rows_c,
                                             ps.rowany_c, st->n_grp_c * (rows_c / 64), ps.grp_any_c, st->n_grp_c, q_bound, walk_scale);
                }
            }
        } else {
            HIPCHK(hipMemsetAsync(ps.ncand, 0, (size_t)n_sub * n_sp * 4, hs));
        }
        seq = ++st->cand_seq;
        skx::launch_cand_publish(hs, st->d_cbad, force_full, ps.ncand, st->d_nqc, d_nd, (u32)n_sub, n_sp, rows_c, ps.mode, ps.any_full,
                                 ps.nqc_total, ps.h_pub, seq);
        if (ranked && P > 0 && !all_forced)
            skx::launch_cand_gather_m(hs, d_m, m_int, n_pad, d_nd, sdm ? ref->n_sd : q_bound, ps.cand, st->n_pad_c, st->d_cbad, (u32)n_sub, ps.mc, rows_c / 64);
        only_if = ps.any_full;
        HIPCHK(hipGetLastError());
    }
    if (P > 0) {
        static const int direct_env = skx::knob("SKX_RARE_DIRECT") ? atoi(skx::knob("SKX_RARE_DIRECT")) : 1;
        const bool direct_rare = split_dict && ref->rare_direct && (direct_env != 0 || sdm);
        if (split_dict && !direct_rare) {
            Span sp(st, 1, hs);
            skx::launch_sparse_fill(hs, st->d_sslot, d_nd, st->rare_index(), d_m, n_pad, d_mdirty, q_bound, only_if);
        }
        if (!direct_rare) HIPCHK(hipMemsetAsync(st->d_mqext + 2 * b, 0, 8, hs));
        {
            Span sp(st, 3, hs);
            skx::launch_transpose_bits(hs, d_m, split ? st->d_mint : nullptr, n_pad, n_words, d_mq, direct_rare ? d_nd + 2 : d_nd + 3, d_grp_any,
                                       nullptr, st->d_wb[b], d_win, ref->n_tiles, d_mdirty, direct_rare ? nd_est : nq_est, st->d_rowany[b], only_if,
                                       sdm && st->reuse_m);
            if (direct_rare)
                skx::launch_rare_to_mq(hs, st->d_sslot, d_nd, st->rare_index(), d_mq, nq_rows, n_pad, st->d_rowany[b], d_grp_any, q_bound, only_if,
                                       st->d_mqext + 2 * b);
            if (only_if && !(sdm && st->reuse_m)) skx::launch_m_clear(hs, d_m, split ? st->d_mint : nullptr, n_pad, d_nd, only_if);
        }
        if (sdm) st->m_ready[b] = false;
    }
    HIPCHK(hipGetLastError());
    HIPCHK(hipEventRecord(st->ev_front[b], hs));
    st->front_pending[b] = true;
    (void)lean_used;

    SKXCHK(queue_chains(st, false));
    skx_stream::PassChains& pc = st->pcq[(st->pc_head + st->pc_n) & 1];
    st->pc_n += 1;
    pc.pending = true; pc.ranked = ranked; pc.has_cand = update_table;
    pc.n_sub = n_sub; pc.b = b; pc.slot = slot; pc.P = P; pc.nq_rows = nq_rows; pc.seq = seq; pc.nq_est = nq_est;
    for (int i = 0; i < n_sub; ++i) pc.subs[i] = subs[i];
    pc.update_table = update_table;
    pc.forced_full = all_forced || legacy;
    pc.legacy = legacy;
    if (legacy) { pc.has_cand = false; all_forced = true; }
    SKX_MARK("pass: scan + transpose queued", 0);
    if (all_forced) SKXCHK(queue_chains(st, true));
// ... 1248 lines not shown
    SKXCHK(flush_pending(st));
    const u32 n = st->ref->n_genomes;
    std::vector<u64> cur(n);
    skx::launch_gather_table(st->hs2, st->d_cum, st->d_tab_tmp, n, st->ref->d_real2pad);
    HIPCHK(hipGetLastError());
    HIPCHK(hipMemcpyAsync(cur.data(), st->d_tab_tmp, (size_t)n * 8, hipMemcpyDeviceToHost, st->hs2));
    HIPCHK(hipStreamSynchronize(st->hs2));
    for (u32 g = 0; g < n; ++g)
        if (cur[g] > SKX_MAX_TABLE_SUM || add[g] > SKX_MAX_TABLE_SUM - cur[g])
            return fail(SKX_ERR_INVALID, "skx_stream_table_add: genome %u would hold more than 2^54 - 1 = 18014398509481983", g);
    HIPCHK(hipMemcpyAsync(st->d_tab_tmp, add, (size_t)n * 8, hipMemcpyHostToDevice, st->hs2));
    skx::launch_add_table(st->hs2, st->d_cum, st->d_tab_tmp, n, st->ref->d_real2pad);
    st->fresh_table = false;
    HIPCHK(hipGetLastError());
    HIPCHK(hipStreamSynchronize(st->hs2));
    return SKX_OK;
}
SKX_API int skx_stream_reset(skx_stream* st) {
    if (!st) return fail(SKX_ERR_INVALID, "NULL stream");
    SKXCHK(use_device(st->device));
    SKXCHK(flush_pending(st));
    HIPCHK(hipStreamSynchronize(st->hs0));
    HIPCHK(hipStreamSynchronize(st->hs1));
    HIPCHK(hipStreamSynchronize(st->hs));
    HIPCHK(hipMemsetAsync(st->d_cum, 0, (size_t)st->ref->n_pad * 8, st->hs2));
    HIPCHK(hipStreamSynchronize(st->hs2));
    st->reads_total = 0;
    st->h_nq[2] = 1; st->h_nq[3] = 1;
    st->hint_all_overflow = false;
    st->hint_seq = st->cand_seq;
    st->legacy_run = 0;
    st->lcount_floor = st->lcount_seq;
    st->fresh_table = true;
    st->cum_writer = nullptr;
    return SKX_OK;
}
SKX_API int skx_stream_reads(const skx_stream* st, uint64_t* n_reads) {
    if (!st || !n_reads) return fail(SKX_ERR_INVALID, "NULL argument");
    *n_reads = st->reads_total;
    for (int i = 0; i < st->n_pend; ++i) *n_reads += st->pend[i].n_reads;
    return SKX_OK;
}
SKX_API int skx_stream_stats(skx_stream* st, uint64_t* out, uint32_t n_out) {
    if (!st || !out) return fail(SKX_ERR_INVALID, "NULL argument");
    uint64_t live = 0;
    SKXCHK(use_device(st->device));
    SKXCHK(skx_stream_sync(st));
    {
        const u32 n_grp = st->ref->n_pad / (skx::kRankWords * 64);
        std::vector<u32> flags(n_grp, 0);
        HIPCHK(hipMemcpy(flags.data(), st->d_grp_any[st->buf ^ 1], (size_t)n_grp * 4, hipMemcpyDeviceToHost));
        for (u32 f : flags) live += f ? 1 : 0;
    }
    const uint64_t v[SKX_N_STATS] = {st->last_pairs, st->last_passes, (uint64_t)(st->ref->d_kt_key ? st->h_nd[2 * (st->buf ^ 1)] : st->h_nq[st->buf ^ 1]), st->reads_big,
                                     st->total_passes, st->lean_passes, st->pcap, live, st->reads_split, st->segs_split, st->pool_grown,
                                     st->shared_passes, st->groups_unshared, st->qcap, st->qrows_grown,
                                     (uint64_t)(st->ref->d_kt_key ? st->h_nd[2 * (st->buf ^ 1) + 1] : st->h_nq[st->buf ^ 1]),
                                     st->batches_compact, st->batches_full};
    for (uint32_t i = 0; i < n_out; ++i) out[i] = i < SKX_N_STATS ? v[i] : 0;
    return SKX_OK;
}
SKX_API int skx_stream_rank(skx_stream* st, uint32_t top_k, uint32_t* idx, uint64_t* sum) {
    if (!st || !idx || !sum) return fail(SKX_ERR_INVALID, "NULL argument");
    const skx_ref* ref = st->ref;
    if (top_k < 1 || top_k > ref->min_species) return fail(SKX_ERR_INVALID, "top_k=%u outside 1..n_genomes", top_k);
    SKXCHK(use_device(st->device));
    SKXCHK(flush_pending(st));
    const size_t rows = (size_t)ref->n_species * top_k;
    if (rows > st->rank_cap) {
        HIPCHK(hipStreamSynchronize(st->hs2));
        (void)hipFree(st->d_rank_idx); (void)hipFree(st->d_rank_sum);
        st->d_rank_idx = nullptr; st->d_rank_sum = nullptr; st->rank_cap = 0;
        HIPCHK(hipMalloc(&st->d_rank_idx, rows * 4));
        HIPCHK(hipMalloc(&st->d_rank_sum, rows * 8));
        st->rank_cap = (u32)rows;
    }
    skx::launch_rank_table(st->hs2, st->d_cum, ref->species(), top_k, st->d_rank_idx, st->d_rank_sum);
    HIPCHK(hipGetLastError());
    HIPCHK(hipMemcpyAsync(idx, st->d_rank_idx, rows * 4, hipMemcpyDeviceToHost, st->hs2));
    HIPCHK(hipMemcpyAsync(sum, st->d_rank_sum, rows * 8, hipMemcpyDeviceToHost, st->hs2));
    HIPCHK(hipStreamSynchronize(st->hs2));
    return SKX_OK;
}

SKX_API int skx_sketch_reads(int device, uint32_t k, uint64_t seed, uint32_t s, const uint8_t* bases,
                             const uint64_t* offsets, uint32_t n_reads, uint64_t* sketches, uint32_t* sketch_len) {
    if (!offsets || !sketches || !sketch_len) return fail(SKX_ERR_INVALID, "NULL argument");
    if (k < 1 || k > SKX_MAX_K || s < 1) return fail(SKX_ERR_INVALID, "bad k/s");
    if (n_reads == 0) return SKX_OK;
    SKXCHK(use_device(device));
    const u64 base0 = offsets[0], n_bases = offsets[n_reads] - base0;
    if (n_bases && !bases) return fail(SKX_ERR_INVALID, "bases is NULL");
    std::vector<u64> off(n_reads + 1);
    u64 longest = 1;
    for (u32 r = 0; r <= n_reads; ++r) {
        off[r] = offsets[r] - base0;
        if (r && offsets[r] < offsets[r - 1]) return fail(SKX_ERR_INVALID, "offsets not monotonic at read %u", r - 1);
        if (r) longest = std::max<u64>(longest, offsets[r] - offsets[r - 1]);
    }
    const u32 stride = (u32)std::min<u64>(s, std::max<u64>(longest, 1));
    uint8_t* d_b = nullptr; u64 *d_o = nullptr, *d_sk = nullptr; u32 *d_len = nullptr, *d_cnt = nullptr, *d_lists = nullptr;
    int rc = SKX_OK;
    hipError_t e = hipSuccess;
    do {
        if ((e = hipMalloc(&d_b, std::max<u64>(n_bases, 1))) != hipSuccess) break;
        if ((e = hipMalloc(&d_o, ((size_t)n_reads + 1) * 8)) != hipSuccess) break;
        if ((e = hipMalloc(&d_sk, (size_t)n_reads * stride * 8)) != hipSuccess) break;
        if ((e = hipMalloc(&d_len, (size_t)n_reads * 4)) != hipSuccess) break;
        if ((e = hipMalloc(&d_cnt, (size_t)n_reads * 4)) != hipSuccess) break;
        if ((e = hipMalloc(&d_lists, 2 * ((size_t)n_reads + 1) * 4)) != hipSuccess) break;
        if (n_bases && (e = hipMemcpy(d_b, bases + base0, n_bases, hipMemcpyHostToDevice)) != hipSuccess) break;
// ... 642 lines not shown
```

sketchy_amd/csrc/skx_kernels.hip:

```cpp
#include <algorithm>
#include <cstdlib>
#include <mutex>
#include <type_traits>

#include "skx_common.hpp"
#include "skx_kernels.hpp"

#ifndef SKX_FEW_CANDS
#define SKX_FEW_CANDS 8
#endif
#ifndef SKX_SCAN_ROWS
#define SKX_SCAN_ROWS 8
#endif
#ifndef SKX_SCAN_OCC
#define SKX_SCAN_OCC 1
#endif
#ifndef SKX_SCAN_SPLIT_READS
#define SKX_SCAN_SPLIT_READS 1
#endif
#ifndef SKX_WALK_BLOCKS
#define SKX_WALK_BLOCKS 256
#endif
#ifndef SKX_GAIN_SPARSE_STRIDE
#define SKX_GAIN_SPARSE_STRIDE 16
// ... 1351 lines not shown
    }
}

__global__ __launch_bounds__(256) void collect_dense_kernel(const u64* __restrict__ key, const u32* __restrict__ off, u64 slots,
                                                            u64* __restrict__ out, u32* __restrict__ out_slot, u32* __restrict__ n, u32 cap) {
    for (u64 i = (u64)blockIdx.x * 256u + threadIdx.x; i < slots; i += (u64)gridDim.x * 256u) {
        const u64 k = key[i];
        if (k == kPad || off[i] != kRareDense) continue;
        const u32 at = atomicAdd(n, 1u);
        if (at < cap) { out[at] = k; out_slot[at] = (u32)i; }
    }
}
__global__ void window_seg_kernel(const u64* __restrict__ lo, const u64* __restrict__ hi, u32 n_bt, u32 n_tiles,
                                  const u64* __restrict__ q, const u32* __restrict__ seg, const u32* __restrict__ grp_sp, u32* __restrict__ win) {
    const u32 bt = blockIdx.x * blockDim.x + threadIdx.x;
    if (bt >= n_bt) return;
    const u32 sp = grp_sp[(bt % n_tiles) / (kRankWords * 64u / kTileGenomes)];
    const u32 a = seg[2u * sp], n = seg[2u * sp + 1u];
    u32 qa = a + n, qb = a + n;
    if (lo[bt] <= hi[bt]) { qa = a + lower_bound_u64(q + a, n, lo[bt]); qb = a + upper_bound_u64(q + a, n, hi[bt]); }
    win[2 * bt] = qa;
    win[2 * bt + 1] = qb;
}
constexpr u32 kCtrStride = 16;
constexpr u32 kShortList = 8;
constexpr u32 kLongFlag = 0x80000000u;
__global__ __launch_bounds__(256) void mlong_build_kernel(const u32* __restrict__ lslot, u32 n_long, const u32* __restrict__ off,
                                                          const u32* __restrict__ cnt, const u32* __restrict__ post, u64* __restrict__ mlong,
                                                          u32 n_gw) {
    const u32 w = blockIdx.x * 4u + (threadIdx.x >> 6), lane = lane_id();
    if (w >= n_long) return;
    const u32 slot = lslot[w], o = off[slot], n = cnt[slot];
    for (u32 j = lane; j < n; j += 64u) {
        const u32 g = post[o + j];
        atomicOr(&mlong[(size_t)w * n_gw + (g >> 6)], 1ull << (g & 63u));
    }
}

__device__ __forceinline__ u64 transpose64(u64 x, u32 lane);
__global__ __launch_bounds__(256) void mlong_transpose_kernel(const u64* __restrict__ mlong, u32 n_long, u32 n_gw, u64* __restrict__ mlongT,
                                                              u32 n_lw) {
    const u32 lw = blockIdx.x, gw = blockIdx.y * 4u + (threadIdx.x >> 6), lane = lane_id();
    if (gw >= n_gw) return;
    const u32 row = lw * 64u + lane;
    const u64 x = row < n_long ? mlong[(size_t)row * n_gw + gw] : 0ull;
    const u64 y = transpose64(x, lane);
    mlongT[((size_t)gw * 64u + lane) * n_lw + lw] = y;
}
constexpr u32 kPatFlag = 0x40000000u;
constexpr u32 kLenMask = 0x3FFFFFFFu;
constexpr u32 kPatNone = 0xFFFFFFFFu;
constexpr u32 kPatRec = 16;
constexpr u32 kPatExcMax = kPatRec - 2u;
__device__ __forceinline__ u32 mix32(u32 x) {
    x = (x ^ (x >> 16)) * 0x7FEB352Du;
    x = (x ^ (x >> 15)) * 0x846CA68Bu;
    return x ^ (x >> 16);
}
__global__ __launch_bounds__(256) void list_sig_kernel(const u32* __restrict__ lslot, u32 n_long, const u32* __restrict__ off,
                                                       const u32* __restrict__ cnt, const u32* __restrict__ post, u32* __restrict__ sig,
                                                       u64* __restrict__ content) {
    const u32 w = blockIdx.x * 4u + (threadIdx.x >> 6), lane = lane_id();
    if (w >= n_long) return;
    const u32 slot = lslot[w], o = off[slot], n = cnt[slot];
    u32 m = 0xFFFFFFFFu;
    u64 c = 0;
    for (u32 j = lane; j < n; j += 64u) {
        const u32 g = post[o + j], x = mix32(g);
        m = min(m, x);
        c += ((u64)x * 0x9E3779B97F4A7C15ull) ^ ((u64)g << 32);
    }
#pragma unroll
    for (int d = 32; d > 0; d >>= 1) { m = min(m, (u32)__shfl_xor((int)m, d, 64)); c += shfl_xor64(c, d); }
    if (lane == 0u) { sig[w] = m; content[w] = c; }
}
__global__ __launch_bounds__(256) void pat_exceptions_kernel(const u64* __restrict__ mlong, u32 n_gw, u32 n_long, const u32* __restrict__ pat_of,
                                                             const u32* __restrict__ pat_rep, u32* __restrict__ prec, u32* __restrict__ n_done) {
    const u32 w = blockIdx.x * 4u + (threadIdx.x >> 6), lane = lane_id();
    if (w >= n_long) return;
    u32* rec = prec + (size_t)w * kPatRec;
    const u32 pat = pat_of[w];
    if (pat == kPatNone) { if (lane == 0u) rec[0] = kPatNone; return; }
    const u64* a = mlong + (size_t)w * n_gw;
    const u64* b = mlong + (size_t)pat_rep[pat] * n_gw;
    u32 total = 0;
    for (u32 i = lane; i < n_gw; i += 64u) total += (u32)__popcll(a[i] ^ b[i]);
#pragma unroll
    for (int d = 32; d > 0; d >>= 1) total += (u32)__shfl_xor((int)total, d, 64);
    if (total > kPatExcMax) { if (lane == 0u) rec[0] = kPatNone; return; }
    u32 at = 0;
    for (u32 i0 = 0; i0 < n_gw; i0 += 64u) {
        const u32 i = i0 + lane;
        const u64 bw = i < n_gw ? b[i] : 0ull;
        u64 x = i < n_gw ? (a[i] ^ bw) : 0ull;
        u64 bal = __ballot(x != 0ull);
        while (bal) {
            const u32 src = (u32)__builtin_ctzll(bal);
            bal &= bal - 1ull;
            u64 xs = readlane64(x, (int)src);
            const u64 bs = readlane64(bw, (int)src);
            while (xs) {
                const u32 bit = (u32)__builtin_ctzll(xs);
                xs &= xs - 1ull;
                if (lane == 0u) rec[2u + at] = ((i0 + src) * 64u + bit) | (((bs >> bit) & 1ull) ? 0x80000000u : 0u);
                ++at;
            }
        }
    }
    if (lane == 0u) { rec[0] = pat; rec[1] = total; atomicAdd(n_done, 1u); }
}
__global__ __launch_bounds__(256) void pat_matrix_kernel(const u64* __restrict__ mlong, const u32* __restrict__ pat_rep, u32 n_pat, u32 n_gw,
                                                         u64* __restrict__ pm, u32 n_pad) {
    const u32 pw = blockIdx.x, gw = blockIdx.y * 4u + (threadIdx.x >> 6), lane = lane_id();
    if (gw >= n_gw) return;
    const u32 p = pw * 64u + lane;
    const u64 x = p < n_pat ? mlong[(size_t)pat_rep[p] * n_gw + gw] : 0ull;
    pm[(size_t)pw * n_pad + gw * 64u + lane] = transpose64(x, lane);
}
__global__ __launch_bounds__(256) void classify_a_kernel(const u64* __restrict__ q, const u32* __restrict__ n_q, RareIndex ri,
                                                         u32* __restrict__ qinfo, u32* __restrict__ qloc, u32* __restrict__ bsum) {
    __builtin_amdgcn_s_setprio(3);
    __shared__ u32 wtot[4];
    const u32 nq = *n_q;
    const u32 q0 = blockIdx.x * 1024u + threadIdx.x * 4u;
    if (blockIdx.x * 1024u >= nq) return;
    u32 c[4], e[4], info[4];
#pragma unroll
    for (int j = 0; j < 4; ++j) {
        c[j] = 0; info[j] = kSlotNone;
        if (q0 + j < nq) {
            const u64 h = q[q0 + j];
            if (h >= kEmpty) c[j] = 1u;
            else {
                u32 slot = kt_start(h, ri.mask);
                for (;;) {
                    const u64 kk = ri.key[slot];
                    if (kk == h) { info[j] = slot; c[j] = ri.off[slot] == kRareDense ? 1u : 0u; break; }
                    if (kk == kPad) break;
                    slot = (slot + 1u) & ri.mask;
                }
            }
        }
    }
    const u32 total = block256_excl_scan4(c, e, wtot);
#pragma unroll
    for (int j = 0; j < 4; ++j)
        if (q0 + j < nq) { qinfo[q0 + j] = info[j]; qloc[q0 + j] = e[j] | (c[j] << 31); }
    if (threadIdx.x == 0) bsum[blockIdx.x] = total;
}
constexpr u32 kNoStatic = 0xFFFFFFFFu;
__global__ __launch_bounds__(1024) void classify_b_kernel(u32* __restrict__ bsum, const u32* __restrict__ n_q, u32* __restrict__ n_d,
                                                          volatile u32* __restrict__ h_words, u32 static_nd) {
    __builtin_amdgcn_s_setprio(3);
    __shared__ u32 part[1024];
    const u32 nq = *n_q, nb = (nq + 1023u) / 1024u, t = threadIdx.x;
    const u32 per = (nb + 1023u) / 1024u;
    u32 mine = 0;
    for (u32 i = 0; i < per; ++i) { const u32 b = t * per + i; if (b < nb) mine += bsum[b]; }
    part[t] = mine;
    __syncthreads();
    for (u32 d = 1; d < 1024u; d <<= 1) {
        const u32 v = t >= d ? part[t - d] : 0u;
// ... 2062 lines not shown
        const u32* c = cnt + (size_t)w * 64u;
        for (u32 j = 0; j < rows; ++j) {
            const u32 bit = j < 32u ? __builtin_amdgcn_ubfe(lo, j, 1u) : __builtin_amdgcn_ubfe(hi, j - 32u, 1u);
#pragma unroll
            for (u32 b = 0; b < NB; ++b) acc[b] += __umul24(bit, c[(size_t)b * row_stride + j]);
        }
    }
#pragma unroll
    for (u32 b = 0; b < NB; ++b)
        if (acc[b]) atomicAdd(&gain[(size_t)b * n_pad + g], acc[b]);
}
__global__ __launch_bounds__(256) void gain_sparse_kernel(const u32* __restrict__ sslot, const u32* __restrict__ n_d, RareIndex ri,
                                                          const u32* __restrict__ cnt, u32 row_stride, u32 n_b, u32 n_pad,
                                                          u32* __restrict__ gain, LongRows lr, PatRows pr) {
    __builtin_amdgcn_s_setprio(2);
    const u32 nd64 = n_d[2], ns = n_d[1], lane = lane_id();
    const u32 wave = blockIdx.x * 4u + (threadIdx.x >> 6), n_waves = gridDim.x * 4u;
    for (u32 r0 = wave * 64u; r0 < ns; r0 += n_waves * 64u) {
        const u32 sr = r0 + lane;
        u32 off = 0, np = 0;
        u32 c[kPassBatchesMax];
        u32 any = 0;
#pragma unroll
        for (u32 b = 0; b < kPassBatchesMax; ++b) c[b] = 0;
        if (sr < ns) {
            const uint2 e = reinterpret_cast<const uint2*>(sslot)[sr];
            off = e.x; np = e.y;
            if (np) {
#pragma unroll
                for (u32 b = 0; b < kPassBatchesMax; ++b)
                    if (b < n_b) { c[b] = cnt[(size_t)b * row_stride + nd64 + sr]; any |= c[b]; }
            }
        }
        const bool is_pat = pr.hist != nullptr && (np & (kLongFlag | kPatFlag)) == (kLongFlag | kPatFlag);
        if (__ballot(is_pat)) {
            u64 bal[kPassBatchesMax];
            u32 mine = 0;
#pragma unroll
            for (u32 b = 0; b < kPassBatchesMax; ++b) {
                bal[b] = __ballot(b < n_b && is_pat && c[b] != 0u);
                if (lane == b) mine = (u32)__popcll(bal[b]);
            }
            u32 base = 0;
            if (mine) base = atomicAdd(&pr.nprow[lane * kCtrStride], mine);
#pragma unroll
            for (u32 b = 0; b < kPassBatchesMax; ++b) {
                const u32 bb = (u32)__shfl((int)base, (int)b);
                if ((bal[b] >> lane) & 1ull)
                    lr.lrow[(size_t)b * lr.lrow_stride + (lr.lrow_stride - 1u - (bb + (u32)__popcll(bal[b] & lanemask_lt())))] = make_uint2(off, sr);
            }
            if (is_pat && any) {
                const u32* rec = ri.prec + (size_t)off * kPatRec;
                const uint4 r0 = *reinterpret_cast<const uint4*>(rec);
                const u32 pat = r0.x, n_exc = r0.y;
#pragma unroll
                for (u32 b = 0; b < kPassBatchesMax; ++b)
                    if (c[b]) atomicAdd(&pr.hist[(size_t)b * pr.hist_stride + pat], c[b]);
                for (u32 j = 0; j < n_exc; ++j) {
                    const u32 e = j == 0u ? r0.z : j == 1u ? r0.w : rec[2u + j];
                    const u32 g = e & 0x7FFFFFFFu;
                    const bool neg = (e >> 31) != 0u;
#pragma unroll
                    for (u32 b = 0; b < kPassBatchesMax; ++b)
                        if (c[b]) atomicAdd(&pr.gain_x[(size_t)b * n_pad + g], neg ? 0u - c[b] : c[b]);
                }
            }
        }
        const bool is_long = (np & kLongFlag) != 0u && !is_pat;
        if (is_pat) np = 0;
        if (__ballot(is_long)) {
            if (lr.lrow) {
                u64 bal[kPassBatchesMax];
                u32 mine = 0;
#pragma unroll
                for (u32 b = 0; b < kPassBatchesMax; ++b) {
                    bal[b] = __ballot(b < n_b && is_long && c[b] != 0u);
                    if (lane == b) mine = (u32)__popcll(bal[b]);
                }
                u32 base = 0;
                if (mine) base = atomicAdd(&lr.nlrow[lane * kCtrStride], mine);
#pragma unroll
                for (u32 b = 0; b < kPassBatchesMax; ++b) {
                    const u32 bb = (u32)__shfl((int)base, (int)b);
                    if ((bal[b] >> lane) & 1ull) {
                        lr.lrow[(size_t)b * lr.lrow_stride + bb + (u32)__popcll(bal[b] & lanemask_lt())] = make_uint2(off, sr);
                        if (lr.inb) atomicOr(&lr.inb[(size_t)b * lr.n_lw + (off >> 6)], 1ull << (off & 63u));
                    }
                }
            }
            if (is_long) np = 0;
        }
        if (!any) np = 0;
        if (np && np <= 8u) {
            for (u32 j = 0; j < np; ++j) {
                const u32 g = ri.post[off + j];
#pragma unroll
                for (u32 b = 0; b < kPassBatchesMax; ++b)
                    if (c[b]) atomicAdd(&gain[((size_t)b * n_pad + g) * kGainSparseStride], c[b]);
            }
        }
        u64 longs = __ballot(np > 8u);
        while (longs) {
            const u32 src = (u32)__builtin_ctzll(longs);
            longs &= longs - 1ull;
            const u32 o = __shfl(off, (int)src), n = __shfl(np, (int)src);
            u32 cc[kPassBatchesMax];
#pragma unroll
            for (u32 b = 0; b < kPassBatchesMax; ++b) cc[b] = __shfl(c[b], (int)src);
            for (u32 j = lane; j < n; j += 64u) {
                const u32 g = ri.post[o + j];
#pragma unroll
                for (u32 b = 0; b < kPassBatchesMax; ++b)
// ... 176 lines not shown
        if (cr == kCandNone) return;
        if (in_lds) {
            for (u32 w = lane; w < n_gw_c; w += 64u) pw[w] = 0ull;
            wave_sync();
        }
        for (u32 k0 = 0; k0 < nw; k0 += 64u) {
            const u32 k = k0 + lane;
            if (k < nw) {
                const u32 wg = wl[k];
                const u64 cm = cwb[wg];
                u64 bits = mrow[wg] & cm;
                const u32 s0 = cbb[wg];
                while (bits) {
                    const u32 bit = (u32)__builtin_ctzll(bits);
                    bits &= bits - 1ull;
                    const u32 slot = s0 + (u32)__popcll(cm & ((1ull << bit) - 1ull));
                    if (in_lds) atomicOr(&pw[slot >> 6], 1ull << (slot & 63u));
                    else atomicOr(&mqc[(size_t)b * mqc_stride + mq_index(slot >> 6, cr, rows_c)], 1ull << (slot & 63u));
                }
            }
        }
        if (in_lds) {
            wave_sync();
            for (u32 w0 = 0; w0 < n_gw_c; w0 += 64u) {
                const u32 w = w0 + lane;
                const u64 v = w < n_gw_c ? pw[w] : 0ull;
                if (v) mqc[(size_t)b * mqc_stride + mq_index(w, cr, rows_c)] = v;
                const u64 nzw = __ballot(v != 0ull);
                const u32 l0 = (lane / kRankWords) * kRankWords;
                if (lane == l0 && w < n_gw_c && ((nzw >> l0) & ((1ull << kRankWords) - 1ull)) != 0ull) {
                    const u32 grp = w / kRankWords;
                    atomicOr(&rowany_c[(size_t)b * rowany_stride + (size_t)grp * (rows_c >> 6) + (cr >> 6)], 1ull << (cr & 63u));
                    u32* ga = grp_any_c + (size_t)b * n_grp_c + grp;
                    if (*ga == 0u) atomicOr(ga, 1u);
                }
            }
            wave_sync();
        } else {
            for (u32 grp = lane; grp < n_grp_c; grp += 64u) {
                atomicOr(&rowany_c[(size_t)b * rowany_stride + (size_t)grp * (rows_c >> 6) + (cr >> 6)], 1ull << (cr & 63u));
                u32* ga = grp_any_c + (size_t)b * n_grp_c + grp;
                if (*ga == 0u) atomicOr(ga, 1u);
            }
        }
    }
}
__global__ void pat_nqc_init_kernel(u32* __restrict__ nqc, u32 v) {
    if (threadIdx.x < kPassBatchesMax) nqc[threadIdx.x * kCtrStride] = v;
}
__global__ __launch_bounds__(256) void cand_pat_rows_kernel(RareIndex ri, const u32* __restrict__ n_d, const u32* __restrict__ candmask,
                                                            const u32* __restrict__ candslot, u32 n_pad, u32* __restrict__ bad,
                                                            u64* __restrict__ pcw, u64* __restrict__ mqc, size_t mqc_stride, u32 rows_c,
                                                            u64* __restrict__ rowany_c, u32 rowany_stride, u32* __restrict__ grp_any_c,
                                                            u32 n_grp_c) {
    __builtin_amdgcn_s_setprio(2);
    __shared__ u64 pat[4][kPatWords];
    const u32 b = blockIdx.y, lane = lane_id(), wv = threadIdx.x >> 6, p = blockIdx.x * 4u + wv;
    if (p >= ri.n_pat || bad[b]) return;
    const u32 nd64 = n_d[2], n_gw_c = n_grp_c * kRankWords, npat64 = (ri.n_pat + 63u) & ~63u;
    if (nd64 + npat64 + 64u >= rows_c) { if (lane == 0u) atomicOr(&bad[b], 2u); return; }
    const u32 cr = nd64 + p;
    u64* pw = pat[wv];
    for (u32 w = lane; w < n_gw_c; w += 64u) pw[w] = 0ull;
    wave_sync();
    const u32 slot = ri.lslot[ri.pat_rep[p]], o = ri.off[slot], n = ri.cnt[slot];
    for (u32 j = lane; j < n; j += 64u) {
        const u32 g = ri.post[o + j];
        if ((candmask[g] >> b) & 1u) {
            const u32 s_ = candslot[(size_t)b * n_pad + g];
            atomicOr(&pw[s_ >> 6], 1ull << (s_ & 63u));
        }
    }
    wave_sync();
    u64* out = pcw + ((size_t)b * ri.n_pat + p) * n_gw_c;
    for (u32 w0 = 0; w0 < n_gw_c; w0 += 64u) {
        const u32 w = w0 + lane;
        const u64 v = w < n_gw_c ? pw[w] : 0ull;
        if (w < n_gw_c) out[w] = v;
        if (v) mqc[(size_t)b * mqc_stride + mq_index(w, cr, rows_c)] = v;
        const u64 nzw = __ballot(v != 0ull);
        const u32 l0 = (lane / kRankWords) * kRankWords;
        if (lane == l0 && w < n_gw_c && ((nzw >> l0) & ((1ull << kRankWords) - 1ull)) != 0ull) {
            const u32 grp = w / kRankWords;
            atomicOr(&rowany_c[(size_t)b * rowany_stride + (size_t)grp * (rows_c >> 6) + (cr >> 6)], 1ull << (cr & 63u));
            u32* ga = grp_any_c + (size_t)b * n_grp_c + grp;
            if (*ga == 0u) atomicOr(ga, 1u);
        }
    }
}
__global__ __launch_bounds__(256) void cand_pat_map_kernel(LongRows lr, PatRows pr, RareIndex ri, const u32* __restrict__ n_d,
                                                           const u32* __restrict__ candmask, const u32* __restrict__ candslot, u32 n_pad,
                                                           u32* __restrict__ bad, u32* __restrict__ nqc, u32* __restrict__ smap, u32 smap_stride,
                                                           const u64* __restrict__ pcw, u64* __restrict__ mqc, size_t mqc_stride, u32 rows_c,
                                                           u64* __restrict__ rowany_c, u32 rowany_stride, u32* __restrict__ grp_any_c,
                                                           u32 n_grp_c) {
    __builtin_amdgcn_s_setprio(2);
    const u32 b = blockIdx.y;
    if (bad[b]) return;
    const u32 nd64 = n_d[2], nr = pr.nprow[b * kCtrStride], n_gw_c = n_grp_c * kRankWords;
    for (u32 i = blockIdx.x * 256u + threadIdx.x; i < nr; i += gridDim.x * 256u) {
        const uint2 e = lr.lrow[(size_t)b * lr.lrow_stride + (lr.lrow_stride - 1u - i)];
        const u32* rec = ri.prec + (size_t)e.x * kPatRec;
        const u32 p = rec[0], n_exc = rec[1];
        u32 fl[kPatExcMax];
        u32 nf = 0;
#pragma unroll
        for (u32 j = 0; j < kPatExcMax; ++j) {
            fl[j] = kCandNone;
            if (j < n_exc) {
                const u32 g = rec[2u + j] & 0x7FFFFFFFu;
                if ((candmask[g] >> b) & 1u) { fl[j] = candslot[(size_t)b * n_pad + g]; ++nf; }
            }
        }
        if (nf == 0u) { smap[(size_t)b * smap_stride + e.y] = nd64 + p + 1u; continue; }
        const u32 cr = nd64 + atomicAdd(&nqc[b * kCtrStride], 1u);
        if (cr + 1u >= rows_c) { atomicOr(&bad[b], 2u); continue; }
        smap[(size_t)b * smap_stride + e.y] = cr + 1u;
        const u64* src = pcw + ((size_t)b * ri.n_pat + p) * n_gw_c;
        for (u32 grp = 0; grp < n_grp_c; ++grp) {
            u64 any = 0ull;
#pragma unroll
            for (u32 k = 0; k < kRankWords; ++k) {
                const u32 w = grp * kRankWords + k;
                u64 v = src[w];
#pragma unroll
                for (u32 j = 0; j < kPatExcMax; ++j) v ^= (fl[j] >> 6) == w ? 1ull << (fl[j] & 63u) : 0ull;
                if (v) mqc[(size_t)b * mqc_stride + mq_index(w, cr, rows_c)] = v;
                any |= v;
            }
            if (any) {
                atomicOr(&rowany_c[(size_t)b * rowany_stride + (size_t)grp * (rows_c >> 6) + (cr >> 6)], 1ull << (cr & 63u));
                u32* ga = grp_any_c + (size_t)b * n_grp_c + grp;
                if (*ga == 0u) atomicOr(ga, 1u);
            }
        }
    }
}
__global__ __launch_bounds__(256) void pass_tables_kernel(const u64* prev, const u32* __restrict__ gain,
                                                          const u32* __restrict__ gain_s, const u32* __restrict__ gain_l, u32 n_b, u32 n_pad,
                                                          u64* tab) {
    __builtin_amdgcn_s_setprio(3);
    const u32 g = blockIdx.x * 256u + threadIdx.x;
    if (g >= n_pad) return;
    u64 t = prev[g];
    tab[g] = t;
    for (u32 b = 0; b < n_b; ++b) {
        t += gain[(size_t)b * n_pad + g];
        if (gain_s) t += gain_s[((size_t)b * n_pad + g) * kGainSparseStride];
        if (gain_l) t += gain_l[(size_t)b * n_pad + g];
        tab[(size_t)(b + 1u) * n_pad + g] = t;
    }
}

__device__ __forceinline__ u64 block1024_max_u64(u64 v, u64* sh ) {
#pragma unroll
    for (int d = 32; d > 0; d >>= 1) v = max(v, shfl_xor64(v, d));
    __syncthreads();
    if (lane_id() == 0u) sh[threadIdx.x >> 6] = v;
    __syncthreads();
    u64 r = sh[0];
#pragma unroll
    for (int i = 1; i < 16; ++i) r = max(r, sh[i]);
    return r;
}
__device__ __forceinline__ u32 block1024_sum_u32(u32 v, u32* sh ) {
#pragma unroll
    for (int d = 32; d > 0; d >>= 1) v += (u32)__shfl_xor((int)v, d, 64);
    __syncthreads();
    if (lane_id() == 0u) sh[threadIdx.x >> 6] = v;
    __syncthreads();
    u32 r = 0;
#pragma unroll
    for (int i = 0; i < 16; ++i) r += sh[i];
    return r;
}
__device__ __forceinline__ u64 species_theta(const u64* __restrict__ t0, u32 g0, u32 n, u32 top_k, u64* sh64, u32* sh32) {
    const u32 tid = threadIdx.x;
// ... 556 lines not shown
    hipLaunchKernelGGL(classify_c_kernel, dim3(std::max(1u, cdiv(q_bound, 256))), dim3(256), 0, st, q, n_q, qinfo, qloc, bsum, n_d, qd, qrow, sslot, ri);
}
void launch_sparse_fill(hipStream_t st, const u32* sslot, const u32* n_d, const RareIndex& ri, u64* m_bits, u32 n_pad, u32* m_dirty, u32 rows_bound,
                        const u32* only_if) {
    const u32 blocks = std::max(1u, std::min(cdiv(rows_bound, 256), kWalkBlocks));
    hipLaunchKernelGGL(sparse_fill_kernel, dim3(blocks), dim3(256), 0, st, sslot, n_d, ri, m_bits, n_pad, m_dirty, only_if);
}
void launch_rare_to_mq(hipStream_t st, const u32* sslot, const u32* n_d, const RareIndex& ri, u64* mq, u32 nq_rows, u32 n_pad, u64* rowany,
                       u32* grp_any, u32 rows_bound, const u32* only_if, u32* ext) {
    const u32 blocks = std::max(1u, std::min(cdiv(rows_bound, 64), 1024u));
    const u32 chunk = std::min(kRareGrpChunk, std::max(1u, (u32)env_int("SKX_RARE_CHUNK", (int)kRareGrpChunk)));
    static const bool sparse_off = env_int("SKX_RARE_SPARSE_WRITES", 1) == 0;
    hipLaunchKernelGGL(rare_to_mq_kernel, dim3(blocks), dim3(256), 0, st, sslot, n_d, ri, mq, nq_rows, n_pad / 64, rowany, grp_any, only_if, chunk,
                       sparse_off ? nullptr : ext);
    if (ext) hipLaunchKernelGGL(mq_extent_kernel, dim3(1), dim3(1), 0, st, ext, nq_rows, n_d, only_if);
}
u32 mq_any_stride() { return kAnyStride; }
void launch_nd_from_nq(hipStream_t st, const u32* n_q, u32* n_d, u32* h_words) {
    hipLaunchKernelGGL(nd_from_nq_kernel, dim3(1), dim3(1), 0, st, n_q, n_d, h_words);
}
void launch_pass_hist(hipStream_t st, const u32* pair_q, const PassBatches& pb, u32* cnt, u32 row_stride) {
    const u32 n = pb.p_off[pb.n];
    if (n == 0) return;
    hipLaunchKernelGGL(pass_hist_kernel, dim3(cdiv(n, 256)), dim3(256), 0, st, pair_q, pb, cnt, row_stride);
}
void launch_gain_dense(hipStream_t st, const u64* m_bits, const u64* m_int, u32 n_pad, const u32* n_d, u32 rows_bound, const u32* cnt, u32 row_stride,
                       u32 n_b, u32* gain, const u32* segw, const u32* grp_sp) {
    const dim3 grid(n_pad / 256, std::max(1u, cdiv(cdiv(rows_bound, 64), kGainWords)));
#define SKX_GAIN(NB) hipLaunchKernelGGL(gain_dense_kernel<NB>, grid, dim3(256), 0, st, m_bits, m_int, n_pad, n_d, cnt, row_stride, gain, segw, grp_sp)
    switch (n_b) {
        case 1: SKX_GAIN(1); break; case 2: SKX_GAIN(2); break; case 3: SKX_GAIN(3); break; case 4: SKX_GAIN(4); break;
        case 5: SKX_GAIN(5); break; case 6: SKX_GAIN(6); break; case 7: SKX_GAIN(7); break; default: SKX_GAIN(8); break;
    }
#undef SKX_GAIN
}
void launch_gain_sparse(hipStream_t st, const u32* n_d, u32 rows_bound, const u32* cnt, u32 row_stride, u32 n_b, u32 n_pad, u32* gain_s,
                        const u32* sslot, const RareIndex& ri, const LongRows* lr, u32 walk_scale, const PatRows* pr) {
    hipLaunchKernelGGL(gain_sparse_kernel, dim3(std::max(1u, std::min(cdiv(rows_bound, 256), kWalkBlocks * std::max(1u, walk_scale)))), dim3(256), 0, st,
                       sslot, n_d, ri, cnt, row_stride, n_b, n_pad, gain_s, lr ? *lr : LongRows{nullptr, nullptr, 0u},
                       (pr && lr && ri.prec) ? *pr : PatRows{nullptr, 0u, nullptr, nullptr});
}
void launch_list_sig(hipStream_t st, const u32* lslot, u32 n_long, const u32* off, const u32* cnt, const u32* post, u32* sig, u64* content) {
    if (n_long == 0) return;
    hipLaunchKernelGGL(list_sig_kernel, dim3(cdiv(n_long, 4)), dim3(256), 0, st, lslot, n_long, off, cnt, post, sig, content);
}
void launch_pat_exceptions(hipStream_t st, const u64* mlong, u32 n_gw, u32 n_long, const u32* pat_of, const u32* pat_rep, u32* prec, u32* n_done) {
    if (n_long == 0) return;
    hipLaunchKernelGGL(pat_exceptions_kernel, dim3(cdiv(n_long, 4)), dim3(256), 0, st, mlong, n_gw, n_long, pat_of, pat_rep, prec, n_done);
}
void launch_pat_matrix(hipStream_t st, const u64* mlong, const u32* pat_rep, u32 n_pat, u32 n_gw, u64* pm, u32 n_pad) {
    if (n_pat == 0) return;
    hipLaunchKernelGGL(pat_matrix_kernel, dim3(cdiv(n_pat, 64), cdiv(n_gw, 4)), dim3(256), 0, st, mlong, pat_rep, n_pat, n_gw, pm, n_pad);
}
u32 pat_record_words() { return kPatRec; }
u32 pat_words_max() { return kPatWords; }
void launch_pat_nqc_init(hipStream_t st, u32* nqc, u32 v) { hipLaunchKernelGGL(pat_nqc_init_kernel, dim3(1), dim3(64), 0, st, nqc, v); }
void launch_cand_pat_rows(hipStream_t st, const RareIndex& ri, const u32* n_d, const u32* candmask, const u32* candslot, u32 n_pad, u32* bad, u32 n_b,
                          u64* pcw, u64* mqc, size_t mqc_stride, u32 rows_c, u64* rowany_c, u32 rowany_stride, u32* grp_any_c, u32 n_grp_c) {
    if (ri.n_pat == 0) return;
    hipLaunchKernelGGL(cand_pat_rows_kernel, dim3(cdiv(ri.n_pat, 4), n_b), dim3(256), 0, st, ri, n_d, candmask, candslot, n_pad, bad, pcw, mqc, mqc_stride,
                       rows_c, rowany_c, rowany_stride, grp_any_c, n_grp_c);
}
void launch_cand_pat_map(hipStream_t st, const LongRows& lr, const PatRows& pr, const RareIndex& ri, const u32* n_d, const u32* candmask,
                         const u32* candslot, u32 n_pad, u32* bad, u32 n_b, u32* nqc, u32* smap, u32 smap_stride, const u64* pcw, u64* mqc,
                         size_t mqc_stride, u32 rows_c, u64* rowany_c, u32 rowany_stride, u32* grp_any_c, u32 n_grp_c, u32 rows_bound, u32 walk_scale) {
    const u32 blocks = std::max(1u, std::min(cdiv(rows_bound, 256), 64u * std::max(1u, walk_scale)));
    hipLaunchKernelGGL(cand_pat_map_kernel, dim3(blocks, n_b), dim3(256), 0, st, lr, pr, ri, n_d, candmask, candslot, n_pad, bad, nqc, smap, smap_stride,
                       pcw, mqc, mqc_stride, rows_c, rowany_c, rowany_stride, grp_any_c, n_grp_c);
}
u32 gain_sparse_stride() { return kGainSparseStride; }
u32 pass_counter_bytes() { return kPassBatchesMax * kCtrStride * 4u; }
void launch_mlong_build(hipStream_t st, const u32* lslot, u32 n_long, const u32* off, const u32* cnt, const u32* post, u64* mlong, u32 n_gw) {
    if (n_long == 0) return;
    hipLaunchKernelGGL(mlong_build_kernel, dim3(cdiv(n_long, 4)), dim3(256), 0, st, lslot, n_long, off, cnt, post, mlong, n_gw);
}
void launch_long_rows(hipStream_t st, const u32* sslot, const u32* n_d, u32 rows_bound, const u32* cnt, u32 row_stride, u32 n_b, const LongRows& lr) {
    hipLaunchKernelGGL(long_rows_kernel, dim3(std::max(1u, std::min(cdiv(rows_bound, 256), (u32)env_int("SKX_G_LONGROWS", 1024)))), dim3(256), 0, st, sslot, n_d, cnt, row_stride, n_b, lr);
}
void launch_gain_long(hipStream_t st, const LongRows& lr, const RareIndex& ri, const u32* n_d, const u32* cnt, u32 row_stride, u32 n_b, u32 n_pad,
                      u32* gain_l, u32 walk_scale) {
    hipLaunchKernelGGL(gain_long_kernel, dim3(cdiv(ri.n_gw, 64), n_b, (u32)env_int("SKX_G_GAINLONG", 8) * std::min(4u, std::max(1u, walk_scale))), dim3(256), 0, st, lr, ri, n_d, cnt, row_stride, n_pad, gain_l);
}
void launch_mlong_transpose(hipStream_t st, const u64* mlong, u32 n_long, u32 n_gw, u64* mlongT, u32 n_lw) {
    if (n_long == 0) return;
    hipLaunchKernelGGL(mlong_transpose_kernel, dim3(n_lw, cdiv(n_gw, 4)), dim3(256), 0, st, mlong, n_long, n_gw, mlongT, n_lw);
}
void launch_cand_hit(hipStream_t st, const u32* cand, u32 n_pad_c, u32 n_b, const u32* bad, const RareIndex& ri, const u64* inb, u64* hit) {
    hipLaunchKernelGGL(cand_hit_kernel, dim3(cdiv(n_pad_c, 4), n_b), dim3(256), 0, st, cand, n_pad_c, bad, ri, inb, hit);
}
void launch_cand_words(hipStream_t st, const u32* cand, u32 n_pad_c, u32 n_b, u32 n_gw, u64* cw, u32* cbase, u32* cwl, u32* ncwl) {
    hipLaunchKernelGGL(cand_words_kernel, dim3(n_b), dim3(1024), 0, st, cand, n_pad_c, n_gw, cw, cbase, cwl, ncwl);
}
void launch_cand_long(hipStream_t st, const LongRows& lr, const RareIndex& ri, const u32* n_d, const u64* cw, const u32* cbase, const u32* cwl,
                      const u32* ncwl, u32 n_pad_c, u32* bad, u32 n_b, u32* nqc, u32* smap, u32 smap_stride, u64* mqc, size_t mqc_stride,
                      u32 rows_c, u64* rowany_c, u32 rowany_stride, u32* grp_any_c, u32 n_grp_c, u32 walk_scale, const u64* hit) {
    hipLaunchKernelGGL(cand_long_kernel, dim3((u32)env_int("SKX_G_CANDLONG", 192) * std::min(4u, std::max(1u, walk_scale)), n_b), dim3(256), 0, st, lr, ri, n_d, cw, cbase, cwl, ncwl, n_pad_c, bad, nqc, smap, smap_stride, mqc,
                       mqc_stride, rows_c, rowany_c, rowany_stride, grp_any_c, n_grp_c, hit);
}
void launch_pass_tables(hipStream_t st, const u64* prev, const u32* gain, const u32* gain_s, const u32* gain_l, u32 n_b, u32 n_pad, u64* tab) {
    hipLaunchKernelGGL(pass_tables_kernel, dim3(cdiv(n_pad, 256)), dim3(256), 0, st, prev, gain, gain_s, gain_l, n_b, n_pad, tab);
}
void launch_cand_select(hipStream_t st, const u64* tab, u32 n_pad, const Species& sp, u32 n_b, u32 top_k, u32 cap, u32* cand, u32* candslot,
                        u64* tabc, u32* ncand, u32* bad, u32* candmask) {
    hipLaunchKernelGGL(cand_select_kernel, dim3(n_b * sp.n_sp), dim3(1024), 0, st, tab, n_pad, sp, top_k, cap, cand, candslot, tabc, ncand, bad, candmask);
}
void launch_cand_count(hipStream_t st, const u64* t0, const u64* t1, const Species& sp, u32 top_k, u32* h_out, u32 seq) {
    hipLaunchKernelGGL(cand_count_kernel, dim3(1), dim3(1024), 0, st, t0, t1, sp, top_k, nullptr, h_out, seq);
}
void launch_cand_gather_m(hipStream_t st, const u64* m_bits, const u64* m_int, u32 n_pad, const u32* n_d, u32 rows_bound, const u32* cand, u32 n_pad_c,
                          const u32* bad, u32 n_b, u64* mc, u32 words_c) {
    const u32 words = std::min(words_c, std::max(1u, cdiv(rows_bound, 64)));
    hipLaunchKernelGGL(cand_gather_m_kernel, dim3(cdiv(n_pad_c, 256), words, n_b), dim3(256), 0, st, m_bits, m_int, n_pad, n_d, cand, n_pad_c, bad, mc, words_c);
}
void launch_cand_sparse(hipStream_t st, const u32* sslot, const u32* n_d, u32 rows_bound, const RareIndex& ri, const u32* candmask,
// ... 666 lines not shown
```

sketchy_amd/csrc/skx_kernels.hpp:

```cpp
#pragma once
#include <hip/hip_runtime.h>
#include <stddef.h>
#include <stdint.h>

#include <stdlib.h>

namespace skx {
typedef unsigned long long u64;
typedef unsigned int u32;

inline const char* knob(const char* name) {
#ifdef SKX_EXPERIMENTS
    return getenv(name);
#else
    (void)name;
    return nullptr;
#endif
}

constexpr int kSketchCap = 2048;
constexpr u32 kSegLen = 64;
constexpr int kRankWords = 8;

struct Species { const u32* g0; const u32* n; const u32* of_grp; u32 n_sp; };

void launch_ref_tile(hipStream_t st, const u64* src, const u32* eff_len, u64* dst, u32 s, u32 pad_base, u32 g_count);
void launch_band_bounds(hipStream_t st, const u64* mat, u32 s, u32 n_tiles, u32 rb, u32 n_bands, u64* lo, u64* hi);

struct LongReads {
    u32* list;
    u32* seg0;
    u32* seg_tab;
    u32* seg_cnt;
    u64* seg_h;
    u32 segs_cap, long_cap;
};
u32 long_read_split();
u32 long_read_seg_slots();
u32 pool_row_fixed();
u32 chk_words();

struct KmerFilter { const u32* words; u32 shift; };
void launch_kmer_filter_build(hipStream_t st, u64 seed, u64 max_ref, const u64* filt, u32 filt_shift, u32* n_keys ,
                              u32* words , u32 shift);

hipError_t launch_sketch(hipStream_t st, const uint8_t* bases, const u64* offsets, u32 n_reads, u32 k, u64 seed, u32 s,
                         u64 max_ref, bool inrange_only, u64* out_sk, u32 sk_stride, u32* out_len, u32* out_cnt_in,
                         const u64* filt , u32 filt_shift,
                         u32* retry , u32* big , u64 n_bases, u32* chk,
                         int leave_room , bool packed = false,
                         const LongReads* long_reads = nullptr, const KmerFilter* kmer_filter = nullptr ,
                         int phase = 3 ,
                         u32 pool_cap = 0 ,
                         u32 pool_fixed = 0 );
hipError_t launch_sketch_block(hipStream_t st, const uint8_t* bases, const u64* offsets, const u32* big, u32 n_big, u32 k, u64 seed,
                               u32 s, u64 max_ref, bool inrange_only, u64* out_sk, u32 sk_stride, u32* out_len, u32* out_cnt_in,
                               const u64* filt, u32 filt_shift, bool packed = false, u32* chk = nullptr, u32 pool_cap = 0,
                               u32 pool_fixed = 0);
void launch_count_scan(hipStream_t st, const u32* in, u32* out, u32 n, u32* bsum);

struct RareIndex { const u64* key; const u32* off; const u32* cnt; const u32* post; u32 mask;
                   const u64* mlong = nullptr; const u32* lid = nullptr; const u32* lslot = nullptr; u32 n_gw = 0;
                   const u64* mlongT = nullptr; u32 n_lw = 0;
                   const u32* prec = nullptr; const u32* pat_rep = nullptr; const u64* pm = nullptr; const u32* d_npat = nullptr; u32 n_pat = 0;
                   const u64* qs = nullptr; u32 n_sd = 0; const u32* srow = nullptr; u32 tail0 = 0; };
void launch_collect_dense(hipStream_t st, const u64* key, const u32* off, u64 slots, u64* out, u32* out_slot, u32* n, u32 cap);
void launch_window_seg(hipStream_t st, const u64* lo, const u64* hi, u32 n_bt, u32 n_tiles, const u64* q, const u32* seg, const u32* grp_sp, u32* win);
struct PatRows { u32* hist; u32 hist_stride; u32* gain_x; u32* nprow; };
void launch_list_sig(hipStream_t st, const u32* lslot, u32 n_long, const u32* off, const u32* cnt, const u32* post, u32* sig, u64* content);
void launch_pat_exceptions(hipStream_t st, const u64* mlong, u32 n_gw, u32 n_long, const u32* pat_of, const u32* pat_rep, u32* prec, u32* n_done);
void launch_pat_matrix(hipStream_t st, const u64* mlong, const u32* pat_rep, u32 n_pat, u32 n_gw, u64* pm, u32 n_pad);
u32 pat_record_words();
u32 pat_words_max();
struct LongRows { uint2* lrow; u32* nlrow; u32 lrow_stride; u64* inb = nullptr; u32 n_lw = 0; };
u32 pass_counter_bytes();
void launch_mlong_build(hipStream_t st, const u32* lslot, u32 n_long, const u32* off, const u32* cnt, const u32* post, u64* mlong, u32 n_gw);
void launch_long_rows(hipStream_t st, const u32* sslot, const u32* n_d, u32 rows_bound, const u32* cnt, u32 row_stride, u32 n_b, const LongRows& lr);
void launch_gain_long(hipStream_t st, const LongRows& lr, const RareIndex& ri, const u32* n_d, const u32* cnt, u32 row_stride, u32 n_b, u32 n_pad,
                      u32* gain_l, u32 walk_scale = 1);
void launch_mlong_transpose(hipStream_t st, const u64* mlong, u32 n_long, u32 n_gw, u64* mlongT, u32 n_lw);
void launch_cand_hit(hipStream_t st, const u32* cand, u32 n_pad_c, u32 n_b, const u32* bad, const RareIndex& ri, const u64* inb, u64* hit);
void launch_cand_words(hipStream_t st, const u32* cand, u32 n_pad_c, u32 n_b, u32 n_gw, u64* cw, u32* cbase, u32* cwl, u32* ncwl);
void launch_cand_long(hipStream_t st, const LongRows& lr, const RareIndex& ri, const u32* n_d, const u64* cw, const u32* cbase, const u32* cwl,
                      const u32* ncwl, u32 n_pad_c, u32* bad, u32 n_b, u32* nqc, u32* smap, u32 smap_stride, u64* mqc, size_t mqc_stride,
                      u32 rows_c, u64* rowany_c, u32 rowany_stride, u32* grp_any_c, u32 n_grp_c, u32 walk_scale = 1, const u64* hit = nullptr );
void launch_rare_count(hipStream_t st, const u64* mat, u64 n_elems, u64* key, u32* cnt, u32 mask, u32* overflow,
                       u64* spmask = nullptr , const u32* grp_sp = nullptr, u32 s = 0);
void launch_rare_fill(hipStream_t st, const u64* mat, u64 n_elems, u32 s, const u64* key, const u32* off, u32* cursor, u32* post, u32 mask);
void launch_classify(hipStream_t st, const u64* q, const u32* n_q, u32 q_bound, const RareIndex& ri, u32* qinfo, u32* qloc, u32* bsum,
                     u64* qd, u32* n_d, u32* qrow, u32* sslot, u32* h_words);
void launch_rare_to_mq(hipStream_t st, const u32* sslot, const u32* n_d, const RareIndex& ri, u64* mq, u32 nq_rows, u32 n_pad, u64* rowany,
                       u32* grp_any, u32 rows_bound, const u32* only_if, u32* ext);
u32 mq_any_stride();
void launch_sparse_fill(hipStream_t st, const u32* sslot, const u32* n_d, const RareIndex& ri, u64* m_bits, u32 n_pad, u32* m_dirty,
                        u32 rows_bound, const u32* only_if = nullptr );
void launch_nd_from_nq(hipStream_t st, const u32* n_q, u32* n_d, u32* h_words);

static const u32 kPassBatchesMax = 8;
static const u32 kCandCap = 1024;
static const u32 kCandRows = 131072;
struct PassBatches { u32 n; u32 p_off[kPassBatchesMax + 1]; };
void launch_pass_hist(hipStream_t st, const u32* pair_q, const PassBatches& pb, u32* cnt, u32 row_stride);
void launch_gain_dense(hipStream_t st, const u64* m_bits, const u64* m_int , u32 n_pad, const u32* n_d, u32 rows_bound, const u32* cnt,
                       u32 row_stride, u32 n_b, u32* gain, const u32* segw = nullptr ,
                       const u32* grp_sp = nullptr);
void launch_gain_sparse(hipStream_t st, const u32* n_d, u32 rows_bound, const u32* cnt, u32 row_stride, u32 n_b, u32 n_pad, u32* gain_s,
                        const u32* sslot, const RareIndex& ri, const LongRows* lr, u32 walk_scale, const PatRows* pr = nullptr);
void launch_pat_nqc_init(hipStream_t st, u32* nqc, u32 v);
void launch_cand_pat_rows(hipStream_t st, const RareIndex& ri, const u32* n_d, const u32* candmask, const u32* candslot, u32 n_pad, u32* bad, u32 n_b,
                          u64* pcw, u64* mqc, size_t mqc_stride, u32 rows_c, u64* rowany_c, u32 rowany_stride, u32* grp_any_c, u32 n_grp_c);
void launch_cand_pat_map(hipStream_t st, const LongRows& lr, const PatRows& pr, const RareIndex& ri, const u32* n_d, const u32* candmask,
                         const u32* candslot, u32 n_pad, u32* bad, u32 n_b, u32* nqc, u32* smap, u32 smap_stride, const u64* pcw, u64* mqc,
                         size_t mqc_stride, u32 rows_c, u64* rowany_c, u32 rowany_stride, u32* grp_any_c, u32 n_grp_c, u32 rows_bound, u32 walk_scale = 1);
u32 gain_sparse_stride();
void launch_pass_tables(hipStream_t st, const u64* prev, const u32* gain, const u32* gain_s , const u32* gain_l , u32 n_b,
                        u32 n_pad, u64* tab);
void launch_cand_select(hipStream_t st, const u64* tab, u32 n_pad, const Species& sp, u32 n_b, u32 top_k, u32 cap, u32* cand, u32* candslot,
                        u64* tabc, u32* ncand, u32* bad, u32* candmask);
void launch_cand_count(hipStream_t st, const u64* t0, const u64* t1, const Species& sp, u32 top_k, u32* h_out, u32 seq);
void launch_cand_gather_m(hipStream_t st, const u64* m_bits, const u64* m_int , u32 n_pad, const u32* n_d, u32 rows_bound, const u32* cand,
                          u32 n_pad_c, const u32* bad, u32 n_b, u64* mc, u32 words_c);
void launch_cand_sparse(hipStream_t st, const u32* sslot, const u32* n_d, u32 rows_bound, const RareIndex& ri, const u32* candmask,
                        const u32* candslot, u32 n_pad, u32* bad, u32 n_b, u32* nqc, u32* smap, u32 smap_stride, u64* mqc, size_t mqc_stride,
                        u32 rows_c, u64* rowany_c, u32 rowany_stride, u32* grp_any_c, u32 n_grp_c, u32 walk_scale = 1);
void launch_cand_publish(hipStream_t st, const u32* bad, u32 force_full, const u32* ncand, const u32* nqc, const u32* n_d, u32 n_b, u32 n_sp,
                         u32 rows_c, u32* mode, u32* any_full, u32* nqc_total, u32* h_pub, u32 seq);
void launch_m_clear(hipStream_t st, u64* m_bits, u64* m_int , u32 n_pad, const u32* n_d, const u32* any_full);
void launch_cand_pair_rows(hipStream_t st, const u32* pair_q, u32 n_pairs, const u32* n_d, const u32* smap, u32 rows_c, u32* pair_qc);
void launch_cand_rows_back(hipStream_t st, u32* out_idx, u32 n_reads, u32 n_sp, u32 top_k, const u32* cand, u32 cap, const u32* g0);
constexpr u32 kConsensusTopMax = 64;
void launch_consensus_rows(hipStream_t st, const u32* idx, u64 first_row, u64 n_rows, u32 n_sp, u32 top_k, const u32* g0, const u32* codes,
                           u32 n_feat, u32* out, u32 n_code_rows);
constexpr u32 kChangeWidthMax = 4096;
void launch_change_flags(hipStream_t st, const u32* rows, u32 width, u32 ra, u32 rb, u32* flag);
void launch_change_events(hipStream_t st, const u32* flag, u32* pos, u32* bsum, u32 n, u32 cap, u32* n_events, u32* ev_read,
                          const u32* idx, const u64* sum, u32 w_idx, u32* ev_idx, u64* ev_sum, const u32* codes, u32 w_codes, u32* ev_codes);

void launch_pair_q(hipStream_t st, const u64* pair_h, u32 n_pairs, const u64* q, const u32* n_q, u32* pair_q, const u32* qrow ,
                   const u32* bbase, const u32* btot, u64 max_ref );
static const int kPairBaseMax = 7;
struct PairBase { const u32* p[kPairBaseMax] = {}; };
void launch_dict_insert(hipStream_t st, const u64* sk, u32 sk_stride, const u32* poff, u32 r_begin, u32 r_end, u32 p_base,
                        u64* pair_h, u32* pair_r, u64* ht, u32 ht_slots, u32* ctr, u32 pair_cap,
                        const u32* row_off = nullptr ,
                        PairBase base = PairBase());
void launch_dict_rest(hipStream_t st, u64* ht, u32 ht_slots, u64 max_ref, u32* slot_off, u32* bcount, u32* bbase, u32* btot,
                      u32* ctr, u64* q, u32* n_q);
u32 dict_buckets();
void launch_window(hipStream_t st, const u64* lo, const u64* hi, u32 n_bt, const u64* q, const u32* n_q, u32* win,
                   u32* h_nq );
void launch_exceptions(hipStream_t st, const u32* exc_g, const u64* exc_h, u32 n_exc, const u64* q, const u32* n_q,
                       u64* m_bits, u32 n_pad, u32* m_dirty , const u32* qrow = nullptr,
                       u32 row0 = 0 , u32 n_fixed = 0 );

bool scan_lean_applies(u32 n_bands, bool split, bool big_table);
u32 scan_lean_words();
bool scan_lean_wants_slabs();
bool scan_lean_into_m();
u32 scan_run_cap();
void launch_scan(hipStream_t st, const u64* mat, u32 s, u32 n_tiles, u32 rb, u32 n_bands, const u64* q, const u32* win,
                 u64* m_bits, u64* m_int, u32 n_pad, bool big_table, bool lean, u64* hbuf, u32* m_dirty, bool into_m = true, u32 run = 0, bool big_slices = false);
u32 scan_lean_cap(bool big);
void launch_word_bands(hipStream_t st, u32* win, u32 n_tiles, u32 n_bands, const u32* n_q, u32* wb, const u64* lo = nullptr,
// ... 77 lines not shown
```

Before: 150.7 million.

## Encode long posting lists as unions of disjoint patterns plus exceptions

Adds a reference-build step that finds long posting lists not matching a single pattern but coverable by a union of up to several disjoint same-species patterns with few exceptions. These lists are re-encoded as pattern-cover records on the GPU. The candidate map kernel ORs the covered pattern rows, tracking per-pattern 'meets' flags so rows that touch no candidate are skipped. The threshold for 'mostly patterns' is relaxed, which can switch off the transposed long-row matrix. The cost is more host-side build work and extra per-row loads and branches in the map kernel.

Result: no change. 150.4 million (-0.2%).

```diff
diff --git a/include/sketchy_hip.h b/include/sketchy_hip.h
--- a/include/sketchy_hip.h
+++ b/include/sketchy_hip.h
@@ -48,6 +48,7 @@
 int skx_ref_kmer_filter(const skx_ref *ref, uint64_t *n_keys, uint64_t *table_bytes);
 int skx_ref_rare_index(const skx_ref *ref, uint64_t *n_keys, uint64_t *n_rare_keys, uint64_t *n_postings, uint64_t *bytes);
 int skx_ref_patterns(const skx_ref *ref, uint64_t *n_long_lists, uint64_t *n_patterns, uint64_t *n_pattern_lists, uint64_t *bytes);
+int skx_ref_pattern_unions(const skx_ref *ref, uint64_t *n_union_lists, uint32_t *max_cover);
 int skx_ref_static_dense(const skx_ref *ref, int *is_static, uint64_t *n_hashes);
 int skx_ref_pass_bytes(const skx_ref *ref, uint64_t *bytes);
 int skx_ref_set_genotypes(skx_ref *ref, uint32_t n_features, const uint32_t *codes);
@@ -79,7 +80,7 @@
 int skx_stream_table_add(skx_stream *st, const uint64_t *add);
 int skx_stream_reset(skx_stream *st);
 int skx_stream_reads(const skx_stream *st, uint64_t *n_reads);
-#define SKX_N_STATS 18
+#define SKX_N_STATS 19
 int skx_stream_stats(skx_stream *st, uint64_t *out, uint32_t n_out);
 int skx_stream_rank(skx_stream *st, uint32_t top_k, uint32_t *idx, uint64_t *sum);
 void skx_stream_destroy(skx_stream *st);
diff --git a/sketchy_amd/_lib.py b/sketchy_amd/_lib.py
--- a/sketchy_amd/_lib.py
+++ b/sketchy_amd/_lib.py
@@ -28,6 +28,7 @@
     ("skx_ref_kmer_filter", _i, [_vp, C.POINTER(_u64), C.POINTER(_u64)]),
     ("skx_ref_rare_index", _i, [_vp, C.POINTER(_u64), C.POINTER(_u64), C.POINTER(_u64), C.POINTER(_u64)]),
     ("skx_ref_patterns", _i, [_vp, C.POINTER(_u64), C.POINTER(_u64), C.POINTER(_u64), C.POINTER(_u64)]),
+    ("skx_ref_pattern_unions", _i, [_vp, C.POINTER(_u64), C.POINTER(_u32)]),
     ("skx_ref_static_dense", _i, [_vp, C.POINTER(C.c_int), C.POINTER(_u64)]),
     ("skx_ref_create", _i, [_pp, _i, _u32, _u64, _u32, _u32, _u32, _vp, _vp]),
     ("skx_ref_create_multi", _i, [_pp, _i, _u32, _u64, _u32, _u32, _u32, _vp, _vp, _vp]),
diff --git a/sketchy_amd/api.py b/sketchy_amd/api.py
--- a/sketchy_amd/api.py
+++ b/sketchy_amd/api.py
@@ -115,6 +115,12 @@
         v = [C.c_uint64(0) for _ in range(4)]
         _lib.check(_lib.load().skx_ref_patterns(self._h, *[C.byref(x) for x in v]))
         return dict(zip(("long_lists", "patterns", "pattern_lists", "bytes"), [x.value for x in v]))
+
+    @property
+    def pattern_unions(self):
+        n, m = C.c_uint64(0), C.c_uint32(0)
+        _lib.check(_lib.load().skx_ref_pattern_unions(self._h, C.byref(n), C.byref(m)))
+        return dict(union_lists=n.value, max_cover=m.value)
 
     @property
     def static_dense(self):
@@ -333,11 +339,12 @@
         return self.ref.consensus_rows(idx)
 
     def stats(self):
-        v = (C.c_uint64 * 18)()
-        _lib.check(_lib.load().skx_stream_stats(self._h, v, 18))
+        v = (C.c_uint64 * 19)()
+        _lib.check(_lib.load().skx_stream_stats(self._h, v, 19))
         names = ("last_pairs", "last_passes", "dictionary_size", "reads_block_sketcher", "passes", "passes_lean_scan",
                  "pair_capacity", "live_rank_groups", "reads_split_over_waves", "read_segments", "row_pool_grown",
-                 "passes_shared", "groups_unshared", "query_rows", "query_rows_grown", "dictionary_dense", "batches_compact", "batches_full")
+                 "passes_shared", "groups_unshared", "query_rows", "query_rows_grown", "dictionary_dense", "batches_compact", "batches_full",
+                 "union_rows_own")
         return dict(zip(names, [int(x) for x in v]))
 
     def set_profiling(self, on=True):
diff --git a/sketchy_amd/csrc/skx_capi.hip b/sketchy_amd/csrc/skx_capi.hip
--- a/sketchy_amd/csrc/skx_capi.hip
+++ b/sketchy_amd/csrc/skx_capi.hip
@@ -260,6 +260,8 @@
     u64* d_pm = nullptr;
     u32 n_pat = 0;
     u64 n_pat_lists = 0;
+    u64 n_union_lists = 0;
+    u32 max_cover = 0;
     bool rare_direct = false;
     u64* d_qs = nullptr;
     u32* d_nsd = nullptr;
@@ -301,6 +303,117 @@
 
 static const u32 kPatMax = 16384;
 static const u32 kPatGroupMin = 4;
+
+static void build_pattern_unions(skx_ref* r) {
+    static const int uni_env = skx::knob("SKX_PATTERN_UNIONS") ? atoi(skx::knob("SKX_PATTERN_UNIONS")) : 1;
+    r->n_union_lists = 0; r->max_cover = 0;
+    if (!uni_env || !r->d_prec || !r->d_pm || !r->n_pat || r->n_pat > skx::pat_id_max() || !r->d_post || !r->d_lslot) return;
+    const u32 n_long = (u32)r->n_long, n_pad = r->n_pad, n_gw = n_pad / 64, n_pat = r->n_pat, n_pw = (n_pat + 63) / 64;
+    const u32 cover_max = skx::pat_cover_max(), rec_words = skx::pat_record_words();
+    const u64 slots = (u64)r->kt_mask + 1;
+    if (r->n_postings > (1ull << 29)) return;
+    u32 *d_urow = nullptr, *d_ucov = nullptr, *d_done = nullptr;
+    try {
+        std::vector<u32> head(n_long), lslot(n_long), off(slots), cnt(slots), post((size_t)std::max<u64>(r->n_postings, 1));
+        std::vector<u64> pm((size_t)n_pw * n_pad);
+        bool ok = hipMemcpy2D(head.data(), 4, r->d_prec, (size_t)rec_words * 4, 4, n_long, hipMemcpyDeviceToHost) == hipSuccess &&
+                  hipMemcpy(lslot.data(), r->d_lslot, (size_t)n_long * 4, hipMemcpyDeviceToHost) == hipSuccess &&
+                  hipMemcpy(off.data(), r->d_kt_off, slots * 4, hipMemcpyDeviceToHost) == hipSuccess &&
+                  hipMemcpy(cnt.data(), r->d_kt_cnt, slots * 4, hipMemcpyDeviceToHost) == hipSuccess &&
+                  hipMemcpy(post.data(), r->d_post, (size_t)r->n_postings * 4, hipMemcpyDeviceToHost) == hipSuccess &&
+                  hipMemcpy(pm.data(), r->d_pm, pm.size() * 8, hipMemcpyDeviceToHost) == hipSuccess;
+        if (!ok) { (void)hipGetLastError(); return; }
+        std::vector<u32> g_off(n_pad + 1, 0), p_off(n_pat + 1, 0);
+        for (u32 w = 0; w < n_pw; ++w)
+            for (u32 g = 0; g < n_pad; ++g) {
+                u64 bits = pm[(size_t)w * n_pad + g];
+                g_off[g + 1] += (u32)__builtin_popcountll(bits);
+                while (bits) { const u32 p = w * 64 + (u32)__builtin_ctzll(bits); bits &= bits - 1; if (p < n_pat) p_off[p + 1] += 1; }
+            }
+        u64 total = 0;
+        for (u32 g = 0; g < n_pad; ++g) { total += g_off[g + 1]; if (total > (1ull << 28)) return; g_off[g + 1] = (u32)total; }
+        for (u32 p = 0; p < n_pat; ++p) p_off[p + 1] += p_off[p];
+        std::vector<u32> g_pat((size_t)total), p_gen((size_t)total), g_at(g_off.begin(), g_off.end() - 1), p_at(p_off.begin(), p_off.end() - 1);
+        for (u32 w = 0; w < n_pw; ++w)
+            for (u32 g = 0; g < n_pad; ++g) {
+                u64 bits = pm[(size_t)w * n_pad + g];
+                while (bits) {
+                    const u32 p = w * 64 + (u32)__builtin_ctzll(bits);
+                    bits &= bits - 1;
+                    g_pat[g_at[g]++] = p;
+                    if (p < n_pat) p_gen[p_at[p]++] = g;
+                }
+            }
+        std::vector<u32>().swap(g_at); std::vector<u32>().swap(p_at); std::vector<u64>().swap(pm);
+        std::vector<u32> g_sp(n_pad, 0), p_sp(n_pat, 0xFFFFFFFFu);
+        for (u32 sp = 0; sp < r->n_species; ++sp) {
+            const u32 g_end = sp + 1 < r->n_species ? r->sp_g0[sp + 1] : n_pad;
+            for (u32 g = r->sp_g0[sp]; g < g_end && g < n_pad; ++g) g_sp[g] = sp;
+        }
+        for (u32 p = 0; p < n_pat; ++p) {
+            for (u32 j = p_off[p]; j < p_off[p + 1]; ++j) {
+                const u32 sp = g_sp[p_gen[j]];
+                if (j == p_off[p]) p_sp[p] = sp;
+                else if (p_sp[p] != sp) { p_sp[p] = 0xFFFFFFFFu; break; }
+            }
+        }
+        std::vector<u32> votes(n_pat, 0), stamp(n_pad, 0), touched, urow, ucov;
+        std::vector<std::pair<u32, u32>> cands;
+        u32 serial = 0;
+        for (u32 row = 0; row < n_long; ++row) {
+            if (head[row] != 0xFFFFFFFFu) continue;
+            const u32 slot = lslot[row];
+            if (slot >= slots || off[slot] == 0xFFFFFFFFu) continue;
+            const u32 o = off[slot], n = cnt[slot];
+            if ((u64)o + n > r->n_postings || n == 0) continue;
+            touched.clear(); cands.clear();
+            bool one_species = true;
+            const u32 sp0 = post[o] < n_pad ? g_sp[post[o]] : 0xFFFFFFFFu;
+            for (u32 j = 0; j < n; ++j) {
+                const u32 g = post[o + j];
+                if (g >= n_pad || g_sp[g] != sp0) { one_species = false; break; }
+                for (u32 k = g_off[g]; k < g_off[g + 1]; ++k) { const u32 p = g_pat[k]; if (votes[p]++ == 0) touched.push_back(p); }
+            }
+            for (u32 p : touched) {
+                const u32 size = p_off[p + 1] - p_off[p];
+                if (one_species && p_sp[p] == sp0 && (u64)votes[p] * 2 > size) cands.push_back({votes[p], p});
+                votes[p] = 0;
+            }
+            if (cands.size() < 2) continue;
+            std::sort(cands.begin(), cands.end(), [](const std::pair<u32, u32>& a, const std::pair<u32, u32>& b) { return a.first != b.first ? a.first > b.first : a.second < b.second; });
+            ++serial;
+            u32 taken[8], m = 0, covered = 0, sizes = 0;
+            for (const auto& c : cands) {
+                const u32 p = c.second;
+                bool disjoint = true;
+                for (u32 j = p_off[p]; j < p_off[p + 1]; ++j) if (stamp[p_gen[j]] == serial) { disjoint = false; break; }
+                if (!disjoint) continue;
+                for (u32 j = p_off[p]; j < p_off[p + 1]; ++j) stamp[p_gen[j]] = serial;
+                taken[m++] = p; covered += c.first; sizes += p_off[p + 1] - p_off[p];
+                if (m == cover_max) break;
+            }
+            if (m < 2) continue;
+            const u32 n_exc = (n - covered) + (sizes - covered), budget = rec_words - 2 - (m > 2 ? 1 : 0) - (m > 4 ? 1 : 0);
+            if (n_exc > budget) continue;
+            urow.push_back(row);
+            for (u32 i = 0; i < cover_max; ++i) ucov.push_back(i < m ? taken[i] : 0xFFFFFFFFu);
+        }
+        const u32 n_u = (u32)urow.size();
+        if (n_u == 0) return;
+        ok = hipMalloc(&d_urow, (size_t)n_u * 4) == hipSuccess && hipMalloc(&d_ucov, (size_t)n_u * cover_max * 4) == hipSuccess &&
+             hipMalloc(&d_done, 8) == hipSuccess && hipMemset(d_done, 0, 8) == hipSuccess &&
+             hipMemcpy(d_urow, urow.data(), (size_t)n_u * 4, hipMemcpyHostToDevice) == hipSuccess &&
+             hipMemcpy(d_ucov, ucov.data(), (size_t)n_u * cover_max * 4, hipMemcpyHostToDevice) == hipSuccess;
+        if (ok) {
+            skx::launch_cover_exceptions(nullptr, r->d_mlong, n_gw, n_long, n_u, d_urow, d_ucov, n_pat, r->d_pat_rep, r->d_prec, d_done);
+            u32 done[2] = {0, 0};
+            ok = hipGetLastError() == hipSuccess && hipDeviceSynchronize() == hipSuccess && hipMemcpy(done, d_done, 8, hipMemcpyDeviceToHost) == hipSuccess;
+            if (ok) { r->n_union_lists = done[0]; r->max_cover = done[1]; }
+        }
+    } catch (const std::bad_alloc&) {}
+    (void)hipFree(d_urow); (void)hipFree(d_ucov); (void)hipFree(d_done);
+    (void)hipGetLastError();
+}
 static void build_patterns(skx_ref* r) {
     static const int pat_env = skx::knob("SKX_PATTERNS") ? atoi(skx::knob("SKX_PATTERNS")) : 1;
     if (!pat_env || !r->d_mlong || r->n_long < 64 || r->n_long >= 0x7FFFFFFFull) return;
@@ -309,7 +422,7 @@
     u64* d_content = nullptr;
     auto drop = [&]() {
         (void)hipFree(r->d_prec); (void)hipFree(r->d_pat_rep); (void)hipFree(r->d_npat); (void)hipFree(r->d_pm);
-        r->d_prec = r->d_pat_rep = r->d_npat = nullptr; r->d_pm = nullptr; r->n_pat = 0; r->n_pat_lists = 0;
+        r->d_prec = r->d_pat_rep = r->d_npat = nullptr; r->d_pm = nullptr; r->n_pat = 0; r->n_pat_lists = 0; r->n_union_lists = 0; r->max_cover = 0;
         (void)hipGetLastError();
     };
     bool ok = hipMalloc(&d_sig, (size_t)n_long * 4) == hipSuccess && hipMalloc(&d_content, (size_t)n_long * 8) == hipSuccess;
@@ -373,6 +486,7 @@
     } catch (const std::bad_alloc&) { ok = false; }
     (void)hipFree(d_sig); (void)hipFree(d_content); (void)hipFree(d_pat_of); (void)hipFree(d_done);
     if (!ok) drop();
+    else build_pattern_unions(r);
 }
 
 static void build_static_dense(skx_ref* r, const std::vector<u64>& exc_h, const std::vector<u64>* spmask) {
@@ -679,7 +793,7 @@
                     }
                     if (lok) r->n_long = n_long;
                     if (lok) build_patterns(r);
-                    const bool mostly_patterns = lok && r->d_prec && r->n_pat_lists * 10 >= n_long * 9;
+                    const bool mostly_patterns = lok && r->d_prec && (r->n_pat_lists + r->n_union_lists) * 4 >= n_long * 3;
                     static const int mlongt_env = skx::knob("SKX_LONG_ROWS_T") ? atoi(skx::knob("SKX_LONG_ROWS_T")) : 1;
                     if (lok && mlongt_env && (!mostly_patterns || mlongt_env == 2)) {
                         const u32 n_lw = (u32)((n_long + 63) / 64);
@@ -699,7 +813,7 @@
                 (void)hipFree(r->d_mlong); (void)hipFree(r->d_mlongT); (void)hipFree(r->d_lid); (void)hipFree(r->d_lslot);
                 r->d_mlong = r->d_mlongT = nullptr; r->d_lid = r->d_lslot = nullptr; r->n_long = 0; r->n_lw = 0;
                 (void)hipFree(r->d_prec); (void)hipFree(r->d_pat_rep); (void)hipFree(r->d_npat); (void)hipFree(r->d_pm);
-                r->d_prec = r->d_pat_rep = r->d_npat = nullptr; r->d_pm = nullptr; r->n_pat = 0; r->n_pat_lists = 0;
+                r->d_prec = r->d_pat_rep = r->d_npat = nullptr; r->d_pm = nullptr; r->n_pat = 0; r->n_pat_lists = 0; r->n_union_lists = 0; r->max_cover = 0;
                 r->rare_direct = false;
                 ok = false;
             }
@@ -794,6 +908,12 @@
     if (n_patterns) *n_patterns = ref->d_prec ? ref->n_pat : 0;
     if (n_pattern_lists) *n_pattern_lists = ref->d_prec ? ref->n_pat_lists : 0;
     if (bytes) *bytes = ref->d_prec ? ref->n_long * skx::pat_record_words() * 4 + (u64)((ref->n_pat + 63) / 64) * ref->n_pad * 8 + (u64)ref->n_pat * 4 : 0;
+    return SKX_OK;
+}
+SKX_API int skx_ref_pattern_unions(const skx_ref* ref, uint64_t* n_union_lists, uint32_t* max_cover) {
+    if (!ref) return fail(SKX_ERR_INVALID, "NULL argument");
+    if (n_union_lists) *n_union_lists = ref->d_prec ? ref->n_union_lists : 0;
+    if (max_cover) *max_cover = ref->d_prec ? ref->max_cover : 0;
     return SKX_OK;
 }
 SKX_API int skx_ref_static_dense(const skx_ref* ref, int* is_static, uint64_t* n_hashes) {
@@ -953,8 +1073,10 @@
     bool use_pat = false;
     u32 *d_hist = nullptr, *d_nprow = nullptr;
     u64* d_pcw = nullptr;
+    u32 *d_pmeet = nullptr;
+    u32 *d_union_own = nullptr;
     u32 npat_pad = 0;
-    skx::PatRows pat_rows() const { return skx::PatRows{d_hist, npat_pad, d_gain_l, d_nprow}; }
+    skx::PatRows pat_rows() const { return skx::PatRows{d_hist, npat_pad, d_gain_l, d_nprow, d_pmeet, d_union_own}; }
     skx::RareIndex rare_index() const {
         skx::RareIndex ri = ref->rare_index();
         if (!use_pat) { ri.prec = nullptr; ri.n_pat = 0; }
@@ -1147,7 +1269,7 @@
                     st->d_topk_idx, st->d_topk_sum, st->d_cons, st->d_ev.n_events, st->d_ev.ev_read, st->d_ev.ev_idx, st->d_ev.ev_sum, st->d_ev.ev_codes, st->d_tab_tmp, st->d_rank_idx, st->d_rank_sum, st->d_bsum, st->d_grp_any[0],
                     st->d_grp_any[1], st->d_hbuf, st->d_wb[0], st->d_wb[1], st->d_rowany[0], st->d_rowany[1], st->d_mqext,
                     st->d_qd, st->d_qrow, st->d_sslot, st->d_qinfo, st->d_qloc, st->d_cls_bsum, st->d_nd_hs,
-                    st->d_rowcnt, st->d_gain, st->d_gain_s, st->d_candslot, st->d_candmask, st->d_lrow, st->d_nlrow, st->d_gain_l, st->d_cbase, st->d_cwl, st->d_ncwl, st->d_cw, st->d_cbad, st->d_nqc, st->d_spc_g0, st->d_spc_grp, st->d_inb, st->d_hit, st->d_hist, st->d_nprow, st->d_pcw, st->d_ms[0], st->d_ms[1], st->d_mdirty_s};
+                    st->d_rowcnt, st->d_gain, st->d_gain_s, st->d_candslot, st->d_candmask, st->d_lrow, st->d_nlrow, st->d_gain_l, st->d_cbase, st->d_cwl, st->d_ncwl, st->d_cw, st->d_cbad, st->d_nqc, st->d_spc_g0, st->d_spc_grp, st->d_inb, st->d_hit, st->d_hist, st->d_nprow, st->d_pcw, st->d_pmeet, st->d_union_own, st->d_ms[0], st->d_ms[1], st->d_mdirty_s};
     for (auto& q : st->ps) {
         for (void* x : {(void*)q.tab, (void*)q.cand, (void*)q.tabc, (void*)q.ncand, (void*)q.mode, (void*)q.any_full, (void*)q.nqc_total, (void*)q.mc, (void*)q.mqc,
                         (void*)q.rowany_c, (void*)q.grp_any_c, (void*)q.smap, (void*)q.pair_qc, (void*)q.nd}) (void)hipFree(x);
@@ -1604,6 +1726,9 @@
                 SCHK(hipMalloc(&st->d_hist, (size_t)nb * st->npat_pad * 4));
                 SCHK(hipMalloc(&st->d_nprow, skx::pass_counter_bytes()));
                 SCHK(hipMalloc(&st->d_pcw, (size_t)nb * ref->n_pat * st->n_grp_c * skx::kRankWords * 8));
+                SCHK(hipMalloc(&st->d_pmeet, (size_t)nb * ref->n_pat * 4));
+                SCHK(hipMalloc(&st->d_union_own, 4));
+                SCHK(hipMemset(st->d_union_own, 0, 4));
             }
         }
         SCHK(hipMalloc(&st->d_cbad, 64));
@@ -2065,7 +2190,7 @@
                     const skx::RareIndex ri = st->rare_index();
                     skx::launch_cand_pat_rows(hs, ri, d_nd, st->d_candmask, st->d_candslot, n_pad, st->d_cbad, (u32)n_sub, st->d_pcw, ps.mqc,
                                               (size_t)st->n_grp_c * rows_c * skx::kRankWords, rows_c, ps.rowany_c, st->n_grp_c * (rows_c / 64), ps.grp_any_c,
-                                              st->n_grp_c);
+                                              st->n_grp_c, st->d_pmeet);
                     skx::launch_cand_pat_map(hs, st->long_rows(), st->pat_rows(), ri, d_nd, st->d_candmask, st->d_candslot, n_pad, st->d_cbad, (u32)n_sub,
                                              st->d_nqc, ps.smap, qstride, st->d_pcw, ps.mqc, (size_t)st->n_grp_c * rows_c * skx::kRankWords, rows_c,
                                              ps.rowany_c, st->n_grp_c * (rows_c / 64), ps.grp_any_c, st->n_grp_c, q_bound, walk_scale);
@@ -3420,11 +3545,13 @@
         HIPCHK(hipMemcpy(flags.data(), st->d_grp_any[st->buf ^ 1], (size_t)n_grp * 4, hipMemcpyDeviceToHost));
         for (u32 f : flags) live += f ? 1 : 0;
     }
+    u32 union_own = 0;
+    if (st->d_union_own) HIPCHK(hipMemcpy(&union_own, st->d_union_own, 4, hipMemcpyDeviceToHost));
     const uint64_t v[SKX_N_STATS] = {st->last_pairs, st->last_passes, (uint64_t)(st->ref->d_kt_key ? st->h_nd[2 * (st->buf ^ 1)] : st->h_nq[st->buf ^ 1]), st->reads_big,
                                      st->total_passes, st->lean_passes, st->pcap, live, st->reads_split, st->segs_split, st->pool_grown,
                                      st->shared_passes, st->groups_unshared, st->qcap, st->qrows_grown,
                                      (uint64_t)(st->ref->d_kt_key ? st->h_nd[2 * (st->buf ^ 1) + 1] : st->h_nq[st->buf ^ 1]),
-                                     st->batches_compact, st->batches_full};
+                                     st->batches_compact, st->batches_full, union_own};
     for (uint32_t i = 0; i < n_out; ++i) out[i] = i < SKX_N_STATS ? v[i] : 0;
     return SKX_OK;
 }
diff --git a/sketchy_amd/csrc/skx_kernels.hip b/sketchy_amd/csrc/skx_kernels.hip
--- a/sketchy_amd/csrc/skx_kernels.hip
+++ b/sketchy_amd/csrc/skx_kernels.hip
@@ -1427,6 +1427,22 @@
 constexpr u32 kPatNone = 0xFFFFFFFFu;
 constexpr u32 kPatRec = 16;
 constexpr u32 kPatExcMax = kPatRec - 2u;
+constexpr u32 kPatUnion = 0x80000000u;
+constexpr u32 kPatCoverMax = 5;
+constexpr u32 kPatIdMax = 1u << 14;
+struct PatCover { u32 m, x0; u32 p[kPatCoverMax]; };
+__device__ __forceinline__ PatCover pat_cover(u32 head, u32 rec2, u32 rec3) {
+    PatCover c;
+#pragma unroll
+    for (u32 i = 0; i < kPatCoverMax; ++i) c.p[i] = 0u;
+    if (!(head & kPatUnion)) { c.m = 1u; c.x0 = 2u; c.p[0] = head; return c; }
+    c.m = min((head >> 28) & 7u, kPatCoverMax);
+    c.p[0] = head & (kPatIdMax - 1u); c.p[1] = (head >> 14) & (kPatIdMax - 1u);
+    c.x0 = 2u + (c.m > 2u ? 1u : 0u) + (c.m > 4u ? 1u : 0u);
+    if (c.m > 2u) { c.p[2] = rec2 & 0xFFFFu; c.p[3] = rec2 >> 16; }
+    if (c.m > 4u) c.p[4] = rec3;
+    return c;
+}
 __device__ __forceinline__ u32 mix32(u32 x) {
     x = (x ^ (x >> 16)) * 0x7FEB352Du;
     x = (x ^ (x >> 15)) * 0x846CA68Bu;
@@ -1483,6 +1499,78 @@
         }
     }
     if (lane == 0u) { rec[0] = pat; rec[1] = total; atomicAdd(n_done, 1u); }
+}
+__global__ __launch_bounds__(256) void cover_exceptions_kernel(const u64* __restrict__ mlong, u32 n_gw, u32 n_long, u32 n_u,
+                                                               const u32* __restrict__ urow, const u32* __restrict__ ucov, u32 n_pat,
+                                                               const u32* __restrict__ pat_rep, u32* __restrict__ prec, u32* __restrict__ n_done) {
+    const u32 w = blockIdx.x * 4u + (threadIdx.x >> 6), lane = lane_id();
+    if (w >= n_u) return;
+    const u32 row = urow[w];
+    if (row >= n_long) return;
+    u32 pid[kPatCoverMax], rep[kPatCoverMax];
+    u32 m = 0;
+    bool okc = true;
+#pragma unroll
+    for (u32 i = 0; i < kPatCoverMax; ++i) {
+        pid[i] = ucov[(size_t)w * kPatCoverMax + i];
+        rep[i] = row;
+        if (pid[i] != kPatNone && m == i) {
+            if (pid[i] < n_pat && pid[i] < kPatIdMax) { rep[i] = pat_rep[pid[i]]; ++m; }
+            else okc = false;
+        }
+    }
+    u32* rec = prec + (size_t)row * kPatRec;
+    if (!okc || m < 2u || rec[0] != kPatNone) return;
+#pragma unroll
+    for (u32 i = 0; i < kPatCoverMax; ++i) if (rep[i] >= n_long) return;
+    const u32 x0 = 2u + (m > 2u ? 1u : 0u) + (m > 4u ? 1u : 0u), budget = kPatRec - x0;
+    const u64* a = mlong + (size_t)row * n_gw;
+    u32 total = 0, sizes = 0, size_or = 0;
+    for (u32 i = lane; i < n_gw; i += 64u) {
+        u64 o = 0ull;
+#pragma unroll
+        for (u32 k = 0; k < kPatCoverMax; ++k)
+            if (k < m) { const u64 v = mlong[(size_t)rep[k] * n_gw + i]; o |= v; sizes += (u32)__popcll(v); }
+        size_or += (u32)__popcll(o);
+        total += (u32)__popcll(a[i] ^ o);
+    }
+#pragma unroll
+    for (int d = 32; d > 0; d >>= 1) {
+        total += (u32)__shfl_xor((int)total, d, 64);
+        sizes += (u32)__shfl_xor((int)sizes, d, 64);
+        size_or += (u32)__shfl_xor((int)size_or, d, 64);
+    }
+    if (sizes != size_or || total > budget) return;
+    u32 at = 0;
+    for (u32 i0 = 0; i0 < n_gw; i0 += 64u) {
+        const u32 i = i0 + lane;
+        u64 bw = 0ull;
+#pragma unroll
+        for (u32 k = 0; k < kPatCoverMax; ++k)
+            if (k < m && i < n_gw) bw |= mlong[(size_t)rep[k] * n_gw + i];
+        u64 x = i < n_gw ? (a[i] ^ bw) : 0ull;
+        u64 bal = __ballot(x != 0ull);
+        while (bal) {
+            const u32 src = (u32)__builtin_ctzll(bal);
+            bal &= bal - 1ull;
+            u64 xs = readlane64(x, (int)src);
+            const u64 bs = readlane64(bw, (int)src);
+            while (xs) {
+                const u32 bit = (u32)__builtin_ctzll(xs);
+                xs &= xs - 1ull;
+                if (lane == 0u && x0 + at < kPatRec) rec[x0 + at] = ((i0 + src) * 64u + bit) | (((bs >> bit) & 1ull) ? 0x80000000u : 0u);
+                ++at;
+            }
+        }
+    }
+    if (lane == 0u) {
+        if (m > 2u) rec[2] = pid[2] | ((m > 3u ? pid[3] : 0u) << 16);
+        if (m > 4u) rec[3] = pid[4];
+        rec[1] = total;
+        rec[0] = kPatUnion | (m << 28) | (pid[1] << 14) | pid[0];
+        atomicAdd(&n_done[0], 1u);
+        atomicMax(&n_done[1], m);
+    }
 }
 __global__ __launch_bounds__(256) void pat_matrix_kernel(const u64* __restrict__ mlong, const u32* __restrict__ pat_rep, u32 n_pat, u32 n_gw,
                                                          u64* __restrict__ pm, u32 n_pad) {
@@ -3651,12 +3739,19 @@
             if (is_pat && any) {
                 const u32* rec = ri.prec + (size_t)off * kPatRec;
                 const uint4 r0 = *reinterpret_cast<const uint4*>(rec);
-                const u32 pat = r0.x, n_exc = r0.y;
-#pragma unroll
-                for (u32 b = 0; b < kPassBatchesMax; ++b)
-                    if (c[b]) atomicAdd(&pr.hist[(size_t)b * pr.hist_stride + pat], c[b]);
+                const u32 n_exc = r0.y;
+                const PatCover cv = pat_cover(r0.x, r0.z, r0.w);
+#pragma unroll
+                for (u32 i = 0; i < kPatCoverMax; ++i) {
+                    if (i < cv.m) {
+#pragma unroll
+                        for (u32 b = 0; b < kPassBatchesMax; ++b)
+                            if (c[b]) atomicAdd(&pr.hist[(size_t)b * pr.hist_stride + cv.p[i]], c[b]);
+                    }
+                }
                 for (u32 j = 0; j < n_exc; ++j) {
-                    const u32 e = j == 0u ? r0.z : j == 1u ? r0.w : rec[2u + j];
+                    const u32 k = cv.x0 + j;
+                    const u32 e = k == 2u ? r0.z : k == 3u ? r0.w : rec[k];
                     const u32 g = e & 0x7FFFFFFFu;
                     const bool neg = (e >> 31) != 0u;
 #pragma unroll
@@ -3939,7 +4034,7 @@
                                                             const u32* __restrict__ candslot, u32 n_pad, u32* __restrict__ bad,
                                                             u64* __restrict__ pcw, u64* __restrict__ mqc, size_t mqc_stride, u32 rows_c,
                                                             u64* __restrict__ rowany_c, u32 rowany_stride, u32* __restrict__ grp_any_c,
-                                                            u32 n_grp_c) {
+                                                            u32 n_grp_c, u32* __restrict__ pmeet) {
     __builtin_amdgcn_s_setprio(2);
     __shared__ u64 pat[4][kPatWords];
     const u32 b = blockIdx.y, lane = lane_id(), wv = threadIdx.x >> 6, p = blockIdx.x * 4u + wv;
@@ -3960,9 +4055,11 @@
     }
     wave_sync();
     u64* out = pcw + ((size_t)b * ri.n_pat + p) * n_gw_c;
+    u64 meets = 0ull;
     for (u32 w0 = 0; w0 < n_gw_c; w0 += 64u) {
         const u32 w = w0 + lane;
         const u64 v = w < n_gw_c ? pw[w] : 0ull;
+        meets |= v;
         if (w < n_gw_c) out[w] = v;
         if (v) mqc[(size_t)b * mqc_stride + mq_index(w, cr, rows_c)] = v;
         const u64 nzw = __ballot(v != 0ull);
@@ -3974,8 +4071,10 @@
             if (*ga == 0u) atomicOr(ga, 1u);
         }
     }
-}
-__global__ __launch_bounds__(256) void cand_pat_map_kernel(LongRows lr, PatRows pr, RareIndex ri, const u32* __restrict__ n_d,
+    const u64 mb = __ballot(meets != 0ull);
+    if (pmeet && lane == 0u) pmeet[(size_t)b * ri.n_pat + p] = mb ? 1u : 0u;
+}
+__global__ __launch_bounds__(256, 3) void cand_pat_map_kernel(LongRows lr, PatRows pr, RareIndex ri, const u32* __restrict__ n_d,
                                                            const u32* __restrict__ candmask, const u32* __restrict__ candslot, u32 n_pad,
                                                            u32* __restrict__ bad, u32* __restrict__ nqc, u32* __restrict__ smap, u32 smap_stride,
                                                            const u64* __restrict__ pcw, u64* __restrict__ mqc, size_t mqc_stride, u32 rows_c,
@@ -3988,28 +4087,48 @@
     for (u32 i = blockIdx.x * 256u + threadIdx.x; i < nr; i += gridDim.x * 256u) {
         const uint2 e = lr.lrow[(size_t)b * lr.lrow_stride + (lr.lrow_stride - 1u - i)];
         const u32* rec = ri.prec + (size_t)e.x * kPatRec;
-        const u32 p = rec[0], n_exc = rec[1];
+        const uint4 r0 = *reinterpret_cast<const uint4*>(rec);
+        const u32 n_exc = r0.y;
+        const PatCover cv = pat_cover(r0.x, r0.z, r0.w);
         u32 fl[kPatExcMax];
         u32 nf = 0;
 #pragma unroll
         for (u32 j = 0; j < kPatExcMax; ++j) {
             fl[j] = kCandNone;
-            if (j < n_exc) {
-                const u32 g = rec[2u + j] & 0x7FFFFFFFu;
+            if (j < n_exc && cv.x0 + j < kPatRec) {
+                const u32 g = rec[cv.x0 + j] & 0x7FFFFFFFu;
                 if ((candmask[g] >> b) & 1u) { fl[j] = candslot[(size_t)b * n_pad + g]; ++nf; }
             }
         }
-        if (nf == 0u) { smap[(size_t)b * smap_stride + e.y] = nd64 + p + 1u; continue; }
+        u32 p = cv.p[0], nm = 1u;
+        if (cv.m > 1u) {
+            nm = 0u;
+#pragma unroll
+            for (u32 i = 0; i < kPatCoverMax; ++i)
+                if (i < cv.m && pr.pmeet[(size_t)b * ri.n_pat + cv.p[i]]) { p = cv.p[i]; ++nm; }
+            if (nf == 0u && nm == 0u) continue;
+        }
+        if (nf == 0u && nm <= 1u) { smap[(size_t)b * smap_stride + e.y] = nd64 + p + 1u; continue; }
         const u32 cr = nd64 + atomicAdd(&nqc[b * kCtrStride], 1u);
         if (cr + 1u >= rows_c) { atomicOr(&bad[b], 2u); continue; }
         smap[(size_t)b * smap_stride + e.y] = cr + 1u;
-        const u64* src = pcw + ((size_t)b * ri.n_pat + p) * n_gw_c;
+        if (cv.m > 1u && pr.n_own) atomicAdd(pr.n_own, 1u);
+        const u64* src = pcw + (size_t)b * ri.n_pat * n_gw_c;
+        u32 po[kPatCoverMax];
+#pragma unroll
+        for (u32 i = 0; i < kPatCoverMax; ++i) po[i] = cv.p[i] * n_gw_c;
+        const u32 cm = cv.m;
         for (u32 grp = 0; grp < n_grp_c; ++grp) {
             u64 any = 0ull;
 #pragma unroll
             for (u32 k = 0; k < kRankWords; ++k) {
                 const u32 w = grp * kRankWords + k;
-                u64 v = src[w];
+                u64 v = src[po[0] + w];
+                if (cm > 1u) {
+#pragma unroll
+                    for (u32 i = 1; i < kPatCoverMax; ++i)
+                        if (i < cm) v |= src[po[i] + w];
+                }
 #pragma unroll
                 for (u32 j = 0; j < kPatExcMax; ++j) v ^= (fl[j] >> 6) == w ? 1ull << (fl[j] & 63u) : 0ull;
                 if (v) mqc[(size_t)b * mqc_stride + mq_index(w, cr, rows_c)] = v;
@@ -4672,14 +4791,22 @@
     if (n_pat == 0) return;
     hipLaunchKernelGGL(pat_matrix_kernel, dim3(cdiv(n_pat, 64), cdiv(n_gw, 4)), dim3(256), 0, st, mlong, pat_rep, n_pat, n_gw, pm, n_pad);
 }
+void launch_cover_exceptions(hipStream_t st, const u64* mlong, u32 n_gw, u32 n_long, u32 n_u, const u32* urow, const u32* ucov, u32 n_pat,
+                             const u32* pat_rep, u32* prec, u32* n_done) {
+    if (n_u == 0) return;
+    hipLaunchKernelGGL(cover_exceptions_kernel, dim3(cdiv(n_u, 4)), dim3(256), 0, st, mlong, n_gw, n_long, n_u, urow, ucov, n_pat, pat_rep, prec, n_done);
+}
+u32 pat_cover_max() { return kPatCoverMax; }
+u32 pat_id_max() { return kPatIdMax; }
 u32 pat_record_words() { return kPatRec; }
 u32 pat_words_max() { return kPatWords; }
 void launch_pat_nqc_init(hipStream_t st, u32* nqc, u32 v) { hipLaunchKernelGGL(pat_nqc_init_kernel, dim3(1), dim3(64), 0, st, nqc, v); }
 void launch_cand_pat_rows(hipStream_t st, const RareIndex& ri, const u32* n_d, const u32* candmask, const u32* candslot, u32 n_pad, u32* bad, u32 n_b,
-                          u64* pcw, u64* mqc, size_t mqc_stride, u32 rows_c, u64* rowany_c, u32 rowany_stride, u32* grp_any_c, u32 n_grp_c) {
+                          u64* pcw, u64* mqc, size_t mqc_stride, u32 rows_c, u64* rowany_c, u32 rowany_stride, u32* grp_any_c, u32 n_grp_c,
+                          u32* pmeet) {
     if (ri.n_pat == 0) return;
     hipLaunchKernelGGL(cand_pat_rows_kernel, dim3(cdiv(ri.n_pat, 4), n_b), dim3(256), 0, st, ri, n_d, candmask, candslot, n_pad, bad, pcw, mqc, mqc_stride,
-                       rows_c, rowany_c, rowany_stride, grp_any_c, n_grp_c);
+                       rows_c, rowany_c, rowany_stride, grp_any_c, n_grp_c, pmeet);
 }
 void launch_cand_pat_map(hipStream_t st, const LongRows& lr, const PatRows& pr, const RareIndex& ri, const u32* n_d, const u32* candmask,
                          const u32* candslot, u32 n_pad, u32* bad, u32 n_b, u32* nqc, u32* smap, u32 smap_stride, const u64* pcw, u64* mqc,
diff --git a/sketchy_amd/csrc/skx_kernels.hpp b/sketchy_amd/csrc/skx_kernels.hpp
--- a/sketchy_amd/csrc/skx_kernels.hpp
+++ b/sketchy_amd/csrc/skx_kernels.hpp
@@ -66,10 +66,14 @@
                    const u64* qs = nullptr; u32 n_sd = 0; const u32* srow = nullptr; u32 tail0 = 0; };
 void launch_collect_dense(hipStream_t st, const u64* key, const u32* off, u64 slots, u64* out, u32* out_slot, u32* n, u32 cap);
 void launch_window_seg(hipStream_t st, const u64* lo, const u64* hi, u32 n_bt, u32 n_tiles, const u64* q, const u32* seg, const u32* grp_sp, u32* win);
-struct PatRows { u32* hist; u32 hist_stride; u32* gain_x; u32* nprow; };
+struct PatRows { u32* hist; u32 hist_stride; u32* gain_x; u32* nprow; u32* pmeet = nullptr; u32* n_own = nullptr; };
 void launch_list_sig(hipStream_t st, const u32* lslot, u32 n_long, const u32* off, const u32* cnt, const u32* post, u32* sig, u64* content);
 void launch_pat_exceptions(hipStream_t st, const u64* mlong, u32 n_gw, u32 n_long, const u32* pat_of, const u32* pat_rep, u32* prec, u32* n_done);
 void launch_pat_matrix(hipStream_t st, const u64* mlong, const u32* pat_rep, u32 n_pat, u32 n_gw, u64* pm, u32 n_pad);
+void launch_cover_exceptions(hipStream_t st, const u64* mlong, u32 n_gw, u32 n_long, u32 n_u, const u32* urow, const u32* ucov, u32 n_pat,
+                             const u32* pat_rep, u32* prec, u32* n_done);
+u32 pat_cover_max();
+u32 pat_id_max();
 u32 pat_record_words();
 u32 pat_words_max();
 struct LongRows { uint2* lrow; u32* nlrow; u32 lrow_stride; u64* inb = nullptr; u32 n_lw = 0; };
@@ -108,7 +112,8 @@
                         const u32* sslot, const RareIndex& ri, const LongRows* lr, u32 walk_scale, const PatRows* pr = nullptr);
 void launch_pat_nqc_init(hipStream_t st, u32* nqc, u32 v);
 void launch_cand_pat_rows(hipStream_t st, const RareIndex& ri, const u32* n_d, const u32* candmask, const u32* candslot, u32 n_pad, u32* bad, u32 n_b,
-                          u64* pcw, u64* mqc, size_t mqc_stride, u32 rows_c, u64* rowany_c, u32 rowany_stride, u32* grp_any_c, u32 n_grp_c);
+                          u64* pcw, u64* mqc, size_t mqc_stride, u32 rows_c, u64* rowany_c, u32 rowany_stride, u32* grp_any_c, u32 n_grp_c,
+                          u32* pmeet);
 void launch_cand_pat_map(hipStream_t st, const LongRows& lr, const PatRows& pr, const RareIndex& ri, const u32* n_d, const u32* candmask,
                          const u32* candslot, u32 n_pad, u32* bad, u32 n_b, u32* nqc, u32* smap, u32 smap_stride, const u64* pcw, u64* mqc,
                          size_t mqc_stride, u32 rows_c, u64* rowany_c, u32 rowany_stride, u32* grp_any_c, u32 n_grp_c, u32 rows_bound, u32 walk_scale = 1);
```
